# ingonyama-zk/icicle

Measured on NVIDIA H100. Metric: bn254_g1_msm_points_per_s, higher is better.
Workload: dtype u32 limbs (254-bit modular integers, Montgomery arithmetic in IMAD.WIDE chains)

## Files before the change

### icicle_b200/api.py

```python
import copy
import ctypes as C
import enum

import numpy as np

from . import capi
from .capi import IcicleError, MsmConfigC, NttConfigC, VecOpsConfigC, lib, check


class Field(enum.IntEnum):
    BN254_FR = 0
    BN254_FQ = 1
    BLS12_381_FR = 2
    BLS12_381_FQ = 3
    BLS12_377_FR = 4
    BLS12_377_FQ = 5
    BW6_761_FQ = 6
    STARK252 = 7
    BABYBEAR = 8
    KOALABEAR = 9
    M31 = 10
    GOLDILOCKS = 11
    BABYBEAR_EXT4 = 12
    KOALABEAR_EXT4 = 13


FIELD_NAMES = {Field.BN254_FR: "bn254_fr", Field.BN254_FQ: "bn254_fq", Field.BLS12_381_FR: "bls12_381_fr",
               Field.BLS12_381_FQ: "bls12_381_fq", Field.BLS12_377_FR: "bls12_377_fr", Field.BLS12_377_FQ: "bls12_377_fq",
               Field.BW6_761_FQ: "bw6_761_fq", Field.STARK252: "stark252", Field.BABYBEAR: "babybear", Field.KOALABEAR: "koalabear", Field.M31: "m31",
               Field.GOLDILOCKS: "goldilocks"}


class Curve(enum.IntEnum):
    BN254_G1 = 0
    BN254_G2 = 1
    BLS12_381_G1 = 2
    BLS12_381_G2 = 3
    BLS12_377_G1 = 4
    BLS12_377_G2 = 5
    BW6_761_G1 = 6
    BW6_761_G2 = 7
    GRUMPKIN = 8


class NTTDir(enum.IntEnum):
    kForward = 0
    kInverse = 1


class Ordering(enum.IntEnum):
    kNN = 0
    kNR = 1
    kRN = 2
    kRR = 3
    kNM = 4
    kMN = 5


class VecOp(enum.IntEnum):
    ADD = 0
    SUB = 1
    MUL = 2
    ACCUMULATE = 3
    SCALAR_ADD_VEC = 4
    SCALAR_SUB_VEC = 5
    SCALAR_MUL_VEC = 6


def field_limbs(field):
    return lib.b200_field_bytes(int(field)) // 4


def scalar_field(curve):
    return Field(lib.b200_curve_scalar_field(int(curve)))


def affine_limbs(curve):
    return lib.b200_curve_affine_bytes(int(curve)) // 4


def projective_limbs(curve):
    return lib.b200_curve_projective_bytes(int(curve)) // 4


def _is_torch(x):
    return type(x).__module__.startswith("torch")


def is_on_device(x):
    return _is_torch(x) and x.is_cuda


def _ptr(x):
    if _is_torch(x):
        if not x.is_contiguous():
            raise ValueError("device/host tensors must be contiguous")
        return x.data_ptr(), bool(x.is_cuda), x
    a = np.ascontiguousarray(x)
    return a.ctypes.data, False, a


def _out_ptr(x):
    if _is_torch(x):
        return _ptr(x)
    if not isinstance(x, np.ndarray) or not x.flags.c_contiguous or not x.flags.writeable or x.dtype.itemsize != 4:
        raise ValueError("output buffers must be writeable C-contiguous numpy arrays of a 32-bit dtype (uint32 limbs)")
    return x.ctypes.data, False, x


def _stream_handle(stream):
    if stream is None:
        return None
    if hasattr(stream, "cuda_stream"):
        return stream.cuda_stream
    return int(stream)


def device_empty(n_limbs_total, device=None):
    import torch
    return torch.empty(int(n_limbs_total), dtype=torch.int32, device=device or "cuda")


def to_device(host_array, device=None, stream=None):
    import torch
    a = np.ascontiguousarray(host_array, dtype=np.uint32)
    t = torch.empty(a.size, dtype=torch.int32, device=device or "cuda")
    check(lib.b200_copy_to_device(t.data_ptr(), a.ctypes.data, a.nbytes, _stream_handle(stream), 0), "copy_to_device")
    return t.view(*a.shape)


def to_host(dev_tensor, shape=None):
    n = dev_tensor.numel() * dev_tensor.element_size() // 4
    out = np.empty(n, dtype=np.uint32)
    check(lib.b200_copy_to_host(out.ctypes.data, dev_tensor.data_ptr(), out.nbytes, None, 0), "copy_to_host")
    return out.reshape(shape if shape is not None else tuple(dev_tensor.shape))


def set_device(device_id):
    check(lib.b200_set_device(int(device_id)), "set_device")


def get_device_count():
    n = C.c_int(0)
    check(lib.b200_get_device_count(C.byref(n)), "get_device_count")
    return n.value


class MSMConfig:

    def __init__(self, **kw):
        self.stream = None
        self.precompute_factor = 1
        self.c = 0
        self.bitsize = 0
        self.batch_size = 1
        self.are_points_shared_in_batch = True
        self.are_scalars_on_device = False
        self.are_scalars_montgomery_form = False
        self.are_points_on_device = False
        self.are_points_montgomery_form = False
        self.are_results_on_device = False
        self.is_async = False
        self.ext = {}
        for k, v in kw.items():
            if not hasattr(self, k):
                raise TypeError(f"MSMConfig has no field {k}")
            setattr(self, k, v)

    def _c(self):
        c = MsmConfigC()
        lib.b200_msm_default_config(C.byref(c))
        c.stream = _stream_handle(self.stream)
        for k in ("precompute_factor", "c", "bitsize", "batch_size"):
            setattr(c, k, int(getattr(self, k)))
        for k in ("are_points_shared_in_batch", "are_scalars_on_device", "are_scalars_montgomery_form", "are_points_on_device",
                  "are_points_montgomery_form", "are_results_on_device", "is_async"):
            setattr(c, k, 1 if getattr(self, k) else 0)
        c.ext_large_bucket_factor = int(self.ext.get("large_bucket_factor", 0))
        c.ext_nof_chunks = int(self.ext.get("nof_chunks", 0))
        c.ext_is_big_triangle = int(bool(self.ext.get("is_big_triangle", False)))
        return c


def default_msm_config():
    return MSMConfig()


def msm(curve, scalars, bases, msm_size, config=None, results=None):
    cfg = copy.copy(config) if config else MSMConfig()
    sp, s_dev, _ks = _ptr(scalars)
    bp, b_dev, _kb = _ptr(bases)
    cfg.are_scalars_on_device = s_dev
    cfg.are_points_on_device = b_dev
    if results is None:
        if cfg.are_results_on_device:
            results = device_empty(cfg.batch_size * projective_limbs(curve)).view(cfg.batch_size, -1)
        else:
            results = np.zeros((cfg.batch_size, projective_limbs(curve)), dtype=np.uint32)
    rp, r_dev, _kr = _out_ptr(results)
    cfg.are_results_on_device = r_dev
    c = cfg._c()
    check(lib.b200_msm(int(curve), sp, bp, int(msm_size), C.byref(c), rp), "msm")
    return results


def msm_precompute_bases(curve, bases, nof_bases, config, output=None):
    cfg = copy.copy(config)
    bp, b_dev, _kb = _ptr(bases)
    cfg.are_points_on_device = b_dev
    if output is None:
        n = nof_bases * cfg.precompute_factor
        output = (device_empty(n * affine_limbs(curve)).view(n, -1) if cfg.are_results_on_device
                  else np.zeros((n, affine_limbs(curve)), dtype=np.uint32))
    op, o_dev, _ko = _out_ptr(output)
    cfg.are_results_on_device = o_dev
    c = cfg._c()
    check(lib.b200_msm_precompute_bases(int(curve), bp, int(nof_bases), C.byref(c), op), "msm_precompute_bases")
    return output


def ec_sum(curve, points, n, config=None, output=None):
    cfg = config or VecOpsConfig()
    fn, ap, op, c, output = _unary("b200_ec_sum", curve, points, 1, projective_limbs(curve), cfg, output)
    check(fn(int(curve), ap, int(n), C.byref(c), op), "ec_sum")
    return output


def msm_choose_c(curve, msm_size, config=None):
    c = (config or MSMConfig())._c()
    return lib.b200_msm_choose_c(int(curve), int(msm_size), C.byref(c))


def msm_pair_levels(curve, msm_size, c=0, config=None):
    cfg = (config or MSMConfig(c=c))._c()
    return lib.b200_msm_pair_levels(int(curve), int(msm_size), C.byref(cfg))


def shard_range(total, parts, index):
    b, c = C.c_uint64(0), C.c_uint64(0)
    lib.b200_shard_range(int(total), int(parts), int(index), C.byref(b), C.byref(c))
    return b.value, b.value + c.value


def _device_ids(n_devices, device_ids):
    if device_ids is None:
        return int(n_devices), None
    arr = (C.c_int * len(device_ids))(*[int(d) for d in device_ids])
    return len(device_ids), arr


def msm_multi_gpu(curve, scalars, bases, msm_size, config=None, results=None, n_devices=0, device_ids=None):
    cfg = copy.copy(config) if config else MSMConfig()
    sp, s_dev, _ks = _ptr(scalars)
    bp, b_dev, _kb = _ptr(bases)
    if results is None:
        results = np.zeros((cfg.batch_size, projective_limbs(curve)), dtype=np.uint32)
    rp, r_dev, _kr = _out_ptr(results)
    cfg.are_scalars_on_device, cfg.are_points_on_device, cfg.are_results_on_device = s_dev, b_dev, r_dev
    n, ids = _device_ids(n_devices, device_ids)
    c = cfg._c()
    check(lib.b200_msm_multi_gpu(int(curve), sp, bp, int(msm_size), C.byref(c), rp, n, ids), "msm_multi_gpu")
    return results


def ntt_multi_gpu(field, input, size, direction, config=None, output=None, n_devices=0, device_ids=None):
    cfg = copy.copy(config) if config else NTTConfig()
    ip, i_dev, _ki = _ptr(input)
    if output is None:
        output = np.zeros((size * cfg.batch_size, field_limbs(field)), dtype=np.uint32)
    op, o_dev, _ko = _out_ptr(output)
    cfg.are_inputs_on_device, cfg.are_outputs_on_device = i_dev, o_dev
    n, ids = _device_ids(n_devices, device_ids)
    c = cfg._c()
    check(lib.b200_ntt_multi_gpu(int(field), ip, int(size), int(direction), C.byref(c), op, n, ids), "ntt_multi_gpu")
    return output


class NTTConfig:

    def __init__(self, **kw):
        self.stream = None
        self.coset_gen = None
        self.batch_size = 1
        self.columns_batch = False
        self.ordering = Ordering.kNN
        self.are_inputs_on_device = False
        self.are_outputs_on_device = False
        self.is_async = False
        self.ext = {}
        for k, v in kw.items():
            if not hasattr(self, k):
                raise TypeError(f"NTTConfig has no field {k}")
            setattr(self, k, v)

    def _c(self):
        c = NttConfigC()
        lib.b200_ntt_default_config(C.byref(c))
        c.stream = _stream_handle(self.stream)
        self._coset_keep = None
        if self.coset_gen is not None:
            self._coset_keep = np.ascontiguousarray(self.coset_gen, dtype=np.uint32)
            c.coset_gen = self._coset_keep.ctypes.data
        c.batch_size = int(self.batch_size)
        c.columns_batch = 1 if self.columns_batch else 0
        c.are_inputs_on_device = 1 if self.are_inputs_on_device else 0
        c.are_outputs_on_device = 1 if self.are_outputs_on_device else 0
        c.is_async = 1 if self.is_async else 0
        c.ordering = int(self.ordering)
        c.ext_ntt_algorithm = int(self.ext.get("ntt_algorithm", 0))
        c.ext_fast_twiddles = int(bool(self.ext.get("fast_twiddles", False)))
        return c


def default_ntt_config():
    return NTTConfig()


def ntt_init_domain(field, primitive_root, stream=None):
    r = np.ascontiguousarray(primitive_root, dtype=np.uint32)
    check(lib.b200_ntt_init_domain(int(field), r.ctypes.data, _stream_handle(stream)), "ntt_init_domain")


def ntt_release_domain(field):
    check(lib.b200_ntt_release_domain(int(field)), "ntt_release_domain")


def get_root_of_unity_from_domain(field, logn):
    out = np.zeros(field_limbs(field), dtype=np.uint32)
    check(lib.b200_ntt_get_root_of_unity_from_domain(int(field), int(logn), out.ctypes.data), "get_root_of_unity_from_domain")
    return out


def ntt(field, input, size, direction, config=None, output=None):
    cfg = copy.copy(config) if config else NTTConfig()
    ip, i_dev, _ki = _ptr(input)
    cfg.are_inputs_on_device = i_dev
    if output is None:
        n = size * cfg.batch_size * field_limbs(field)
        output = device_empty(n) if cfg.are_outputs_on_device else np.zeros((size * cfg.batch_size, field_limbs(field)), dtype=np.uint32)
    op, o_dev, _ko = _out_ptr(output)
    cfg.are_outputs_on_device = o_dev
    c = cfg._c()
    check(lib.b200_ntt(int(field), ip, int(size), int(direction), C.byref(c), op), "ntt")
    return output


EXTENSION_DEGREE = 4


def ntt_extension(field, input, size, direction, config=None, output=None):
    cfg = copy.copy(config) if config else NTTConfig()
    ip, i_dev, _ki = _ptr(input)
    cfg.are_inputs_on_device = i_dev
    w = field_limbs(field) * EXTENSION_DEGREE
    if output is None:
        n = size * cfg.batch_size * w
        output = device_empty(n) if cfg.are_outputs_on_device else np.zeros((size * cfg.batch_size, w), dtype=np.uint32)
    op, o_dev, _ko = _out_ptr(output)
    cfg.are_outputs_on_device = o_dev
    c = cfg._c()
    check(lib.b200_ntt_extension(int(field), ip, int(size), int(direction), C.byref(c), op), "ntt_extension")
    return output


def ecntt(curve, input, size, direction, config=None, output=None):
    cfg = copy.copy(config) if config else NTTConfig()
    ip, i_dev, _ki = _ptr(input)
    cfg.are_inputs_on_device = i_dev
    w = projective_limbs(curve)
    if output is None:
        n = size * cfg.batch_size * w
        output = device_empty(n) if cfg.are_outputs_on_device else np.zeros((size * cfg.batch_size, w), dtype=np.uint32)
    op, o_dev, _ko = _out_ptr(output)
    cfg.are_outputs_on_device = o_dev
    c = cfg._c()
    check(lib.b200_ecntt(int(curve), ip, int(size), int(direction), C.byref(c), op), "ecntt")
    return output


class VecOpsConfig:

    def __init__(self, **kw):
        self.stream = None
        self.is_a_on_device = False
        self.is_b_on_device = False
        self.is_result_on_device = False
        self.is_async = False
        self.batch_size = 1
        self.columns_batch = False
        for k, v in kw.items():
            if not hasattr(self, k):
                raise TypeError(f"VecOpsConfig has no field {k}")
            setattr(self, k, v)

    def _c(self):
        c = VecOpsConfigC()
        lib.b200_vec_ops_default_config(C.byref(c))
        c.stream = _stream_handle(self.stream)
        c.is_a_on_device = 1 if self.is_a_on_device else 0
        c.is_b_on_device = 1 if self.is_b_on_device else 0
        c.is_result_on_device = 1 if self.is_result_on_device else 0
        c.is_async = 1 if self.is_async else 0
        c.batch_size = int(self.batch_size)
        c.columns_batch = 1 if self.columns_batch else 0
        return c


def _out_like(field, n_elems, on_device):
    if on_device:
        return device_empty(n_elems * field_limbs(field)).view(n_elems, -1)
    return np.zeros((n_elems, field_limbs(field)), dtype=np.uint32)


def _vec2(field, op, a, b, size, config, output):
    cfg = copy.copy(config) if config else VecOpsConfig()
    ap, a_dev, _ka = _ptr(a)
    bp, b_dev, _kb = _ptr(b)
    cfg.is_a_on_device, cfg.is_b_on_device = a_dev, b_dev
    if op == VecOp.ACCUMULATE:
        ap, a_dev, _ka = _out_ptr(a)
        output, op_ptr = a, ap
    else:
        if output is None:
            output = _out_like(field, size * cfg.batch_size, cfg.is_result_on_device)
        op_ptr, o_dev, _ko = _out_ptr(output)
        cfg.is_result_on_device = o_dev
    c = cfg._c()
    check(lib.b200_vec_op(int(field), int(op), ap, bp, int(size), C.byref(c), op_ptr), f"vec_op({VecOp(op).name})")
    return output


def vector_add(field, a, b, size, config=None, output=None):
    return _vec2(field, VecOp.ADD, a, b, size, config, output)


def vector_sub(field, a, b, size, config=None, output=None):
    return _vec2(field, VecOp.SUB, a, b, size, config, output)


def vector_mul(field, a, b, size, config=None, output=None):
    return _vec2(field, VecOp.MUL, a, b, size, config, output)


def vector_accumulate(field, a, b, size, config=None):
    return _vec2(field, VecOp.ACCUMULATE, a, b, size, config, None)


def scalar_add_vec(field, scalar_a, b, size, config=None, output=None):
    return _vec2(field, VecOp.SCALAR_ADD_VEC, scalar_a, b, size, config, output)


def scalar_sub_vec(field, scalar_a, b, size, config=None, output=None):
    return _vec2(field, VecOp.SCALAR_SUB_VEC, scalar_a, b, size, config, output)


def scalar_mul_vec(field, scalar_a, b, size, config=None, output=None):
    return _vec2(field, VecOp.SCALAR_MUL_VEC, scalar_a, b, size, config, output)


def ext_mixed_mul(ext_field, a, b, size, config=None, output=None):
    cfg = copy.copy(config) if config else VecOpsConfig()
    ap, a_dev, _ka = _ptr(a)
    bp, b_dev, _kb = _ptr(b)
    cfg.is_a_on_device, cfg.is_b_on_device = a_dev, b_dev
    if output is None:
        output = _out_like(ext_field, size * cfg.batch_size, cfg.is_result_on_device)
    op, o_dev, _ko = _out_ptr(output)
    cfg.is_result_on_device = o_dev
    c = cfg._c()
    check(lib.b200_ext_mixed_mul(int(ext_field), ap, bp, int(size), C.byref(c), op), "ext_mixed_mul")
    return output


def _unary(fn_name, field_or_curve, a, n_out_elems, limbs, config, output, *extra):
    cfg = copy.copy(config) if config else VecOpsConfig()
    ap, a_dev, _ka = _ptr(a)
    cfg.is_a_on_device = a_dev
    if output is None:
        output = (device_empty(n_out_elems * limbs).view(n_out_elems, -1) if cfg.is_result_on_device
                  else np.zeros((n_out_elems, limbs), dtype=np.uint32))
    op, o_dev, _ko = _out_ptr(output)
    cfg.is_result_on_device = o_dev
    c = cfg._c()
    fn = getattr(lib, fn_name)
    return fn, ap, op, c, output


def vector_inv(field, a, size, config=None, output=None):
    cfg = config or VecOpsConfig()
    fn, ap, op, c, output = _unary("b200_vector_inv", field, a, size * cfg.batch_size, field_limbs(field), cfg, output)
    check(fn(int(field), ap, int(size), C.byref(c), op), "vector_inv")
    return output


def vector_div(field, a, b, size, config=None, output=None):
    cfg = copy.copy(config) if config else VecOpsConfig()
    ap, a_dev, _ka = _ptr(a)
    bp, b_dev, _kb = _ptr(b)
    cfg.is_a_on_device, cfg.is_b_on_device = a_dev, b_dev
    if output is None:
        output = _out_like(field, size * cfg.batch_size, cfg.is_result_on_device)
    op, o_dev, _ko = _out_ptr(output)
    cfg.is_result_on_device = o_dev
    c = cfg._c()
    check(lib.b200_vector_div(int(field), ap, bp, int(size), C.byref(c), op), "vector_div")
    return output


def vector_sum(field, a, size, config=None, output=None):
    cfg = config or VecOpsConfig()
    fn, ap, op, c, output = _unary("b200_vector_sum", field, a, cfg.batch_size, field_limbs(field), cfg, output)
    check(fn(int(field), ap, int(size), C.byref(c), op), "vector_sum")
    return output


def vector_product(field, a, size, config=None, output=None):
    cfg = config or VecOpsConfig()
    fn, ap, op, c, output = _unary("b200_vector_product", field, a, cfg.batch_size, field_limbs(field), cfg, output)
    check(fn(int(field), ap, int(size), C.byref(c), op), "vector_product")
    return output


def highest_non_zero_idx(field, a, size, config=None):
    cfg = copy.copy(config) if config else VecOpsConfig()
    ap, a_dev, _ka = _ptr(a)
    cfg.is_a_on_device = a_dev
    cfg.is_result_on_device = False
    out = np.zeros(cfg.batch_size, dtype=np.int64)
    c = cfg._c()
    check(lib.b200_highest_non_zero_idx(int(field), ap, int(size), C.byref(c), out.ctypes.data), "highest_non_zero_idx")
    return out


def poly_eval(field, coeffs, coeffs_size, domain, domain_size, config=None, output=None):
    cfg = copy.copy(config) if config else VecOpsConfig()
    cp, c_dev, _kc = _ptr(coeffs)
    dp, d_dev, _kd = _ptr(domain)
    cfg.is_a_on_device, cfg.is_b_on_device = c_dev, d_dev
    if output is None:
        output = _out_like(field, domain_size * cfg.batch_size, cfg.is_result_on_device)
    op, o_dev, _ko = _out_ptr(output)
    cfg.is_result_on_device = o_dev
    c = cfg._c()
    check(lib.b200_poly_eval(int(field), cp, int(coeffs_size), dp, int(domain_size), C.byref(c), op), "poly_eval")
    return output


def poly_division(field, numerator, numerator_size, denominator, denominator_size, q_size, r_size, config=None):
    cfg = copy.copy(config) if config else VecOpsConfig()
    n_p, n_dev, _kn = _ptr(numerator)
    d_p, d_dev, _kd = _ptr(denominator)
    cfg.is_a_on_device, cfg.is_b_on_device, cfg.is_result_on_device = n_dev, d_dev, False
    q = np.zeros((q_size * cfg.batch_size, field_limbs(field)), dtype=np.uint32)
    r = np.zeros((r_size * cfg.batch_size, field_limbs(field)), dtype=np.uint32)
    c = cfg._c()
    check(lib.b200_poly_division(int(field), n_p, int(numerator_size), d_p, int(denominator_size), C.byref(c), q.ctypes.data, int(q_size),
                                 r.ctypes.data, int(r_size)), "poly_division")
    return q, r


def convert_montgomery(field, a, size, is_into, config=None, output=None):
    cfg = config or VecOpsConfig()
    fn, ap, op, c, output = _unary("b200_convert_montgomery", field, a, size * cfg.batch_size, field_limbs(field), cfg, output)
    check(fn(int(field), ap, int(size), 1 if is_into else 0, C.byref(c), op), "convert_montgomery")
    return output


def bit_reverse(field, a, size, config=None, output=None):
    cfg = config or VecOpsConfig()
    fn, ap, op, c, output = _unary("b200_bit_reverse", field, a, size * cfg.batch_size, field_limbs(field), cfg, output)
    check(fn(int(field), ap, int(size), C.byref(c), op), "bit_reverse")
    return output


def matrix_transpose(field, a, rows, cols, config=None, output=None):
    cfg = config or VecOpsConfig()
    fn, ap, op, c, output = _unary("b200_matrix_transpose", field, a, rows * cols * cfg.batch_size, field_limbs(field), cfg, output)
    check(fn(int(field), ap, int(rows), int(cols), C.byref(c), op), "matrix_transpose")
    return output


def slice(field, a, offset, stride, size_in, size_out, config=None, output=None):
    cfg = config or VecOpsConfig()
    fn, ap, op, c, output = _unary("b200_slice", field, a, size_out * cfg.batch_size, field_limbs(field), cfg, output)
    check(fn(int(field), ap, int(offset), int(stride), int(size_in), int(size_out), C.byref(c), op), "slice")
    return output


def affine_convert_montgomery(curve, a, n, is_into, config=None, output=None):
    cfg = config or VecOpsConfig()
    fn, ap, op, c, output = _unary("b200_affine_convert_montgomery", curve, a, n, affine_limbs(curve), cfg, output)
    check(fn(int(curve), ap, int(n), 1 if is_into else 0, C.byref(c), op), "affine_convert_montgomery")
    return output


def projective_convert_montgomery(curve, a, n, is_into, config=None, output=None):
    cfg = config or VecOpsConfig()
    fn, ap, op, c, output = _unary("b200_projective_convert_montgomery", curve, a, n, projective_limbs(curve), cfg, output)
    check(fn(int(curve), ap, int(n), 1 if is_into else 0, C.byref(c), op), "projective_convert_montgomery")
    return output


def set_tuning(name, value):
    check(lib.b200_set_tuning(name.encode(), -1 if value is None else int(value)), f"set_tuning({name})")


def get_tuning(name):
    return int(lib.b200_get_tuning(name.encode()))


def trim_scratch(keep_bytes=0):
    check(lib.b200_trim_scratch(int(keep_bytes)), "trim_scratch")


def launch_count():
    return int(lib.b200_get_launch_count())


def set_profiling(on):
    lib.b200_set_profiling(1 if on else 0)


def last_profile():
    names = C.create_string_buffer(2048)
    ms = (C.c_float * 64)()
    k = lib.b200_get_last_profile(names, 2048, ms, 64)
    parts = names.value.decode().split(",")
    return parts[0], [(parts[1 + i], float(ms[i])) for i in range(k)]
```

### icicle_b200/capi.py

```python
import ctypes as C
import os

_HERE = os.path.dirname(os.path.abspath(__file__))
LIB_PATH = os.environ.get("ICICLE_B200_LIB", os.path.join(_HERE, "libicicle_b200.so"))

ERROR_NAMES = {
    0: "SUCCESS", 1: "INVALID_DEVICE", 2: "OUT_OF_MEMORY", 3: "INVALID_POINTER", 4: "ALLOCATION_FAILED",
    5: "DEALLOCATION_FAILED", 6: "COPY_FAILED", 7: "SYNCHRONIZATION_FAILED", 8: "STREAM_CREATION_FAILED",
    9: "STREAM_DESTRUCTION_FAILED", 10: "API_NOT_IMPLEMENTED", 11: "INVALID_ARGUMENT", 12: "BACKEND_LOAD_FAILED",
    13: "LICENSE_CHECK_ERROR", 14: "UNKNOWN_ERROR",
}


class IcicleError(RuntimeError):
    def __init__(self, code, what):
        self.code = code
        super().__init__(f"{what}: eIcicleError::{ERROR_NAMES.get(code, code)}")


class MsmConfigC(C.Structure):
    _fields_ = [
        ("stream", C.c_void_p), ("precompute_factor", C.c_int), ("c", C.c_int), ("bitsize", C.c_int), ("batch_size", C.c_int),
        ("are_points_shared_in_batch", C.c_uint8), ("are_scalars_on_device", C.c_uint8), ("are_scalars_montgomery_form", C.c_uint8),
        ("are_points_on_device", C.c_uint8), ("are_points_montgomery_form", C.c_uint8), ("are_results_on_device", C.c_uint8),
        ("is_async", C.c_uint8), ("reserved", C.c_uint8),
        ("ext_large_bucket_factor", C.c_int), ("ext_nof_chunks", C.c_int), ("ext_is_big_triangle", C.c_int),
    ]


class NttConfigC(C.Structure):
    _fields_ = [
        ("stream", C.c_void_p), ("coset_gen", C.c_void_p), ("batch_size", C.c_int),
        ("columns_batch", C.c_uint8), ("are_inputs_on_device", C.c_uint8), ("are_outputs_on_device", C.c_uint8), ("is_async", C.c_uint8),
        ("ordering", C.c_int), ("ext_ntt_algorithm", C.c_int), ("ext_fast_twiddles", C.c_int),
    ]


class VecOpsConfigC(C.Structure):
    _fields_ = [
        ("stream", C.c_void_p), ("is_a_on_device", C.c_uint8), ("is_b_on_device", C.c_uint8), ("is_result_on_device", C.c_uint8),
        ("is_async", C.c_uint8), ("batch_size", C.c_int), ("columns_batch", C.c_uint8), ("reserved", C.c_uint8 * 3),
    ]


_vp, _i, _u64, _u32, _sz = C.c_void_p, C.c_int, C.c_uint64, C.c_uint32, C.c_size_t
SYMBOLS = {
    "b200_get_device_count": (_i, [C.POINTER(_i)]),
    "b200_set_device": (_i, [_i]),
    "b200_malloc": (_i, [C.POINTER(_vp), _sz]),
    "b200_malloc_async": (_i, [C.POINTER(_vp), _sz, _vp]),
    "b200_free": (_i, [_vp]),
    "b200_free_async": (_i, [_vp, _vp]),
    "b200_get_available_memory": (_i, [C.POINTER(_sz), C.POINTER(_sz)]),
    "b200_memset": (_i, [_vp, _i, _sz]),
    "b200_memset_async": (_i, [_vp, _i, _sz, _vp]),
    "b200_copy_to_device": (_i, [_vp, _vp, _sz, _vp, _i]),
    "b200_copy_to_host": (_i, [_vp, _vp, _sz, _vp, _i]),
    "b200_copy_device_to_device": (_i, [_vp, _vp, _sz, _vp, _i]),
    "b200_synchronize": (_i, [_vp]),
    "b200_create_stream": (_i, [C.POINTER(_vp)]),
    "b200_destroy_stream": (_i, [_vp]),
    "b200_host_alloc_pinned": (_i, [C.POINTER(_vp), _sz]),
    "b200_host_free_pinned": (_i, [_vp]),
    "b200_field_bytes": (_i, [_i]),
    "b200_curve_scalar_field": (_i, [_i]),
    "b200_curve_affine_bytes": (_i, [_i]),
    "b200_curve_projective_bytes": (_i, [_i]),
    "b200_msm_default_config": (None, [C.POINTER(MsmConfigC)]),
    "b200_msm": (_i, [_i, _vp, _vp, _i, C.POINTER(MsmConfigC), _vp]),
    "b200_msm_precompute_bases": (_i, [_i, _vp, _i, C.POINTER(MsmConfigC), _vp]),
    "b200_ec_sum": (_i, [_i, _vp, _i, C.POINTER(VecOpsConfigC), _vp]),
    "b200_msm_choose_c": (_i, [_i, _i, C.POINTER(MsmConfigC)]),
    "b200_msm_pair_levels": (_i, [_i, _i, C.POINTER(MsmConfigC)]),
    "b200_msm_pipeline_schedule": (_i, [_i, C.POINTER(C.c_uint32), _i]),
    "b200_ntt_default_config": (None, [C.POINTER(NttConfigC)]),
    "b200_ntt_init_domain": (_i, [_i, _vp, _vp]),
    "b200_ntt_release_domain": (_i, [_i]),
    "b200_ntt_get_root_of_unity_from_domain": (_i, [_i, _u64, _vp]),
    "b200_ntt": (_i, [_i, _vp, _i, _i, C.POINTER(NttConfigC), _vp]),
    "b200_ntt_extension": (_i, [_i, _vp, _i, _i, C.POINTER(NttConfigC), _vp]),
    "b200_ecntt": (_i, [_i, _vp, _i, _i, C.POINTER(NttConfigC), _vp]),
    "b200_vec_ops_default_config": (None, [C.POINTER(VecOpsConfigC)]),
    "b200_vec_op": (_i, [_i, _i, _vp, _vp, _u64, C.POINTER(VecOpsConfigC), _vp]),
    "b200_ext_mixed_mul": (_i, [_i, _vp, _vp, _u64, C.POINTER(VecOpsConfigC), _vp]),
    "b200_vector_inv": (_i, [_i, _vp, _u64, C.POINTER(VecOpsConfigC), _vp]),
    "b200_vector_div": (_i, [_i, _vp, _vp, _u64, C.POINTER(VecOpsConfigC), _vp]),
    "b200_vector_sum": (_i, [_i, _vp, _u64, C.POINTER(VecOpsConfigC), _vp]),
    "b200_vector_product": (_i, [_i, _vp, _u64, C.POINTER(VecOpsConfigC), _vp]),
    "b200_highest_non_zero_idx": (_i, [_i, _vp, _u64, C.POINTER(VecOpsConfigC), _vp]),
    "b200_poly_eval": (_i, [_i, _vp, _u64, _vp, _u64, C.POINTER(VecOpsConfigC), _vp]),
    "b200_poly_division": (_i, [_i, _vp, _u64, _vp, _u64, C.POINTER(VecOpsConfigC), _vp, _u64, _vp, _u64]),
    "b200_convert_montgomery": (_i, [_i, _vp, _u64, _i, C.POINTER(VecOpsConfigC), _vp]),
    "b200_bit_reverse": (_i, [_i, _vp, _u64, C.POINTER(VecOpsConfigC), _vp]),
    "b200_matrix_transpose": (_i, [_i, _vp, _u32, _u32, C.POINTER(VecOpsConfigC), _vp]),
    "b200_slice": (_i, [_i, _vp, _u64, _u64, _u64, _u64, C.POINTER(VecOpsConfigC), _vp]),
    "b200_affine_convert_montgomery": (_i, [_i, _vp, _u64, _i, C.POINTER(VecOpsConfigC), _vp]),
    "b200_projective_convert_montgomery": (_i, [_i, _vp, _u64, _i, C.POINTER(VecOpsConfigC), _vp]),
    "b200_get_launch_count": (C.c_longlong, []),
    "b200_set_profiling": (None, [_i]),
    "b200_get_last_profile": (_i, [C.c_char_p, _i, C.POINTER(C.c_float), _i]),
    "b200_msm_multi_gpu": (_i, [_i, _vp, _vp, _i, C.POINTER(MsmConfigC), _vp, _i, C.POINTER(_i)]),
    "b200_ntt_multi_gpu": (_i, [_i, _vp, _i, _i, C.POINTER(NttConfigC), _vp, _i, C.POINTER(_i)]),
    "b200_ntt_dist_phase1": (_i, [_i, _vp, _i, _i, _i, _i, _i, _vp]),
    "b200_ntt_dist_phase2": (_i, [_i, _vp, _vp, _i, _i, _i, _i, _i, _vp]),
    "b200_shard_range": (None, [_u64, _i, _i, C.POINTER(_u64), C.POINTER(_u64)]),
    "b200_set_tuning": (_i, [C.c_char_p, _i]),
    "b200_get_tuning": (_i, [C.c_char_p]),
    "b200_trim_scratch": (_i, [_sz]),
    "b200_version": (C.c_char_p, []),
}


def load(path=LIB_PATH):
    if not os.path.exists(path):
        raise ImportError(
            f"icicle_b200: native library not found at {path}. Build it with `python -c 'import __graft_entry__ as g; g.build()'` "
            "or `make -C icicle_b200/csrc`. There is no CPU fallback.")
    lib = C.CDLL(path)
    for name, (res, args) in SYMBOLS.items():
        fn = getattr(lib, name)
        fn.restype = res
        fn.argtypes = args
    return lib


lib = load()


def check(code, what):
    if code != 0:
        raise IcicleError(code, what)
```

### icicle_b200/csrc/common.cuh

```cuda
#pragma once
#include <cuda_runtime.h>
#include <cstdint>
#include <cstdio>
#include <cstdlib>
#include "../../include/icicle_b200.h"
#include "ff.cuh"
#include "ext.cuh"
#include "ext4.cuh"
#include "goldilocks.cuh"
#include "ec.cuh"

namespace b200 {

#define B200_CUDA_TRY(expr, errcode)                                                                                   \
  do {                                                                                                                 \
    cudaError_t _e = (expr);                                                                                           \
    if (_e != cudaSuccess) {                                                                                           \
      fprintf(stderr, "[icicle_b200] %s:%d %s -> %s\n", __FILE__, __LINE__, #expr, cudaGetErrorString(_e));           \
      return (errcode);                                                                                                \
    }                                                                                                                  \
  } while (0)

static inline int map_alloc_error(cudaError_t e) { return e == cudaErrorMemoryAllocation ? B200_OUT_OF_MEMORY : B200_ALLOCATION_FAILED; }

enum Tune : int {
  T_MSM_PAIR_LEVELS = 0, T_MSM_CHUNK_TARGET, T_MSM_NO_WIDE_LOADS, T_MSM_PIPELINE_MIN, T_MSM_PIPELINE_CHUNKS, T_MSM_NO_PIPELINE,
  T_MSM_STAGING_MB, T_MSM_SORT, T_NTT_GEOM, T_NTT31_OFF, T_NTT_COLUMNS_STRIDED, T_NTT_MAXR, T_NTT_TILES, T_NTT_MAXS, T_NTT31_TMA_OFF, T_COPIER_THREADS,
  T_COUNT
};
int tune(Tune k);

cudaMemPool_t scratch_pool();

struct Scratch {
  void* p = nullptr;
  cudaStream_t s = nullptr;
  Scratch() = default;
  Scratch(const Scratch&) = delete;
  Scratch& operator=(const Scratch&) = delete;
  int alloc(size_t bytes, cudaStream_t stream)
  {
    release();
    s = stream;
    if (bytes == 0) bytes = 16;
    cudaMemPool_t pool = scratch_pool();
    cudaError_t e = pool ? cudaMallocFromPoolAsync(&p, bytes, pool, stream) : cudaMallocAsync(&p, bytes, stream);
    if (e != cudaSuccess) {
      p = nullptr;
      fprintf(stderr, "[icicle_b200] scratch allocation of %zu bytes failed: %s\n", bytes, cudaGetErrorString(e));
      (void)cudaGetLastError();
      return map_alloc_error(e);
    }
    return B200_SUCCESS;
  }
  void release()
  {
    if (p) cudaFreeAsync(p, s);
    p = nullptr;
  }
  ~Scratch() { release(); }
  template <class T>
  T* as() const { return reinterpret_cast<T*>(p); }
};

}
#include "hostcopy.cuh"
namespace b200 {

static inline bool ptr_on_device(const void* p, bool flag)
{
  if (flag) return true;
  cudaPointerAttributes a;
  if (cudaPointerGetAttributes(&a, p) != cudaSuccess) {
    (void)cudaGetLastError();
    return false;
  }
  return a.type == cudaMemoryTypeDevice || a.type == cudaMemoryTypeManaged;
}
static inline bool misaligned16(const void* p) { return (((uintptr_t)p) & 15u) != 0; }

static inline int stage_in(const void*& dev_ptr, const void* src, size_t bytes, bool on_device, cudaStream_t s, Scratch& buf)
{
  on_device = ptr_on_device(src, on_device);
  if (on_device && !misaligned16(src)) {
    dev_ptr = src;
    return B200_SUCCESS;
  }
  int err = buf.alloc(bytes, s);
  if (err) return err;
  dev_ptr = buf.p;
  if (!on_device && bytes >= RING_MIN_BYTES && host_kind(src, false) == HK_PAGEABLE) return ring_h2d(buf.p, src, bytes, s);
  B200_CUDA_TRY(cudaMemcpyAsync(buf.p, src, bytes, on_device ? cudaMemcpyDeviceToDevice : cudaMemcpyHostToDevice, s), B200_COPY_FAILED);
  return B200_SUCCESS;
}
static inline int stage_out(void*& dev_ptr, void* dst, size_t bytes, bool on_device, cudaStream_t s, Scratch& buf)
{
  on_device = ptr_on_device(dst, on_device);
  if (on_device && !misaligned16(dst)) {
    dev_ptr = dst;
    return B200_SUCCESS;
  }
  int err = buf.alloc(bytes, s);
  if (err) return err;
  dev_ptr = buf.p;
  return B200_SUCCESS;
}
static inline int finish_out(void* dst, const void* dev_ptr, size_t bytes, bool on_device, bool is_async, cudaStream_t s)
{
  on_device = ptr_on_device(dst, on_device);
  if (dst != dev_ptr && !on_device && bytes >= RING_MIN_BYTES && host_kind(dst, false) == HK_PAGEABLE) return ring_d2h(dst, dev_ptr, bytes, s);
  if (dst != dev_ptr)
    B200_CUDA_TRY(cudaMemcpyAsync(dst, dev_ptr, bytes, on_device ? cudaMemcpyDeviceToDevice : cudaMemcpyDeviceToHost, s), B200_COPY_FAILED);
  if (!on_device || !is_async) B200_CUDA_TRY(cudaStreamSynchronize(s), B200_SYNCHRONIZATION_FAILED);
  return B200_SUCCESS;
}

extern "C" B200_API void b200_count_launch(int n);
#define B200_LAUNCHED(n) b200_count_launch(n)

struct StageTimer {
  static constexpr int MAX_STAGES = 64;
  cudaEvent_t ev[MAX_STAGES + 1];
  const char* names[MAX_STAGES];
  int n = 0;
  bool on = false;
  cudaStream_t s = nullptr;
  void begin(cudaStream_t stream);
  void mark(const char* name);
  void finish(const char* what);
  ~StageTimer();
};

static inline int num_sms()
{
  static thread_local int cached_dev = -1, cached = 132;
  int dev = 0;
  cudaGetDevice(&dev);
  if (dev != cached_dev) {
    cudaDeviceGetAttribute(&cached, cudaDevAttrMultiProcessorCount, dev);
    cached_dev = dev;
  }
  return cached;
}

#define B200_FIELD_CASE(ID, PARAMS, ...)                                                                               \
  case ID: {                                                                                                           \
    using F = ::b200::Fp<::b200::params::PARAMS>;                                                                      \
    __VA_ARGS__;                                                                                                       \
  } break;

#define B200_EXT4_CASE(ID, PARAMS, ...)                                                                                \
  case ID: {                                                                                                           \
    using F = ::b200::Ext4<::b200::params::PARAMS>;                                                                    \
    __VA_ARGS__;                                                                                                       \
  } break;

#define B200_DISPATCH_FIELD(field, ...)                                                                                \
  switch (field) {                                                                                                     \
    B200_FIELD_CASE(B200_FIELD_BN254_FR, bn254_fr, __VA_ARGS__)                                                        \
    B200_FIELD_CASE(B200_FIELD_BN254_FQ, bn254_fq, __VA_ARGS__)                                                        \
    B200_FIELD_CASE(B200_FIELD_BLS12_381_FR, bls12_381_fr, __VA_ARGS__)                                                \
    B200_FIELD_CASE(B200_FIELD_BLS12_381_FQ, bls12_381_fq, __VA_ARGS__)                                                \
    B200_FIELD_CASE(B200_FIELD_BLS12_377_FR, bls12_377_fr, __VA_ARGS__)                                                \
    B200_FIELD_CASE(B200_FIELD_BLS12_377_FQ, bls12_377_fq, __VA_ARGS__)                                                \
    B200_FIELD_CASE(B200_FIELD_BW6_761_FQ, bw6_761_fq, __VA_ARGS__)                                                    \
    B200_FIELD_CASE(B200_FIELD_STARK252, stark252, __VA_ARGS__)                                                        \
    B200_FIELD_CASE(B200_FIELD_BABYBEAR, babybear, __VA_ARGS__)                                                        \
    B200_FIELD_CASE(B200_FIELD_KOALABEAR, koalabear, __VA_ARGS__)                                                      \
    B200_FIELD_CASE(B200_FIELD_M31, m31, __VA_ARGS__)                                                                  \
    B200_FIELD_CASE(B200_FIELD_GOLDILOCKS, goldilocks, __VA_ARGS__)                                                    \
    B200_EXT4_CASE(B200_FIELD_BABYBEAR_EXT4, babybear, __VA_ARGS__)                                                    \
    B200_EXT4_CASE(B200_FIELD_KOALABEAR_EXT4, koalabear, __VA_ARGS__)                                                  \
  default:                                                                                                             \
    return B200_INVALID_ARGUMENT;                                                                                      \
  }

#define B200_DISPATCH_NTT_FIELD(field, ...)                                                                            \
  switch (field) {                                                                                                     \
    B200_FIELD_CASE(B200_FIELD_BN254_FR, bn254_fr, __VA_ARGS__)                                                        \
    B200_FIELD_CASE(B200_FIELD_BLS12_381_FR, bls12_381_fr, __VA_ARGS__)                                                \
    B200_FIELD_CASE(B200_FIELD_BLS12_377_FR, bls12_377_fr, __VA_ARGS__)                                                \
    B200_FIELD_CASE(B200_FIELD_BLS12_377_FQ, bls12_377_fq, __VA_ARGS__)                                                \
    B200_FIELD_CASE(B200_FIELD_STARK252, stark252, __VA_ARGS__)                                                        \
    B200_FIELD_CASE(B200_FIELD_BABYBEAR, babybear, __VA_ARGS__)                                                        \
    B200_FIELD_CASE(B200_FIELD_KOALABEAR, koalabear, __VA_ARGS__)                                                      \
    B200_FIELD_CASE(B200_FIELD_GOLDILOCKS, goldilocks, __VA_ARGS__)                                                    \
  default:                                                                                                             \
    return B200_API_NOT_IMPLEMENTED;                                                                                   \
  }

static inline int field_limbs(int field)
{
  switch (field) {
  case B200_FIELD_BN254_FR: case B200_FIELD_BN254_FQ: case B200_FIELD_BLS12_381_FR: case B200_FIELD_BLS12_377_FR:
  case B200_FIELD_STARK252: return 8;
  case B200_FIELD_BLS12_381_FQ: case B200_FIELD_BLS12_377_FQ: return 12;
  case B200_FIELD_BW6_761_FQ: return 24;
  case B200_FIELD_BABYBEAR: case B200_FIELD_KOALABEAR: case B200_FIELD_M31: return 1;
  case B200_FIELD_GOLDILOCKS: return 2;
  case B200_FIELD_BABYBEAR_EXT4: case B200_FIELD_KOALABEAR_EXT4: return 4;
  default: return 0;
  }
}

template <class FrParams_, class Base_>
struct CurveT {
  typedef FrParams_ FrParams;
  typedef Fp<FrParams_> Scalar;
  typedef Base_ Base;
};

#define B200_CURVE_CASE(ID, FR, BASE, ...)                                                                             \
  case ID: {                                                                                                           \
    using C = ::b200::CurveT<::b200::params::FR, BASE>;                                                                \
    __VA_ARGS__;                                                                                                       \
  } break;

#define B200_DISPATCH_CURVE(curve, ...)                                                                                \
  switch (curve) {                                                                                                     \
    B200_CURVE_CASE(B200_CURVE_BN254_G1, bn254_fr, ::b200::Fp<::b200::params::bn254_fq>, __VA_ARGS__)                  \
    B200_CURVE_CASE(B200_CURVE_BN254_G2, bn254_fr, ::b200::Fp2<::b200::params::bn254_fq>, __VA_ARGS__)                 \
    B200_CURVE_CASE(B200_CURVE_BLS12_381_G1, bls12_381_fr, ::b200::Fp<::b200::params::bls12_381_fq>, __VA_ARGS__)      \
    B200_CURVE_CASE(B200_CURVE_BLS12_381_G2, bls12_381_fr, ::b200::Fp2<::b200::params::bls12_381_fq>, __VA_ARGS__)     \
    B200_CURVE_CASE(B200_CURVE_BLS12_377_G1, bls12_377_fr, ::b200::Fp<::b200::params::bls12_377_fq>, __VA_ARGS__)      \
    B200_CURVE_CASE(B200_CURVE_BLS12_377_G2, bls12_377_fr, ::b200::Fp2<::b200::params::bls12_377_fq>, __VA_ARGS__)     \
    B200_CURVE_CASE(B200_CURVE_BW6_761_G1, bls12_377_fq, ::b200::Fp<::b200::params::bw6_761_fq>, __VA_ARGS__)          \
    B200_CURVE_CASE(B200_CURVE_BW6_761_G2, bls12_377_fq, ::b200::Fp<::b200::params::bw6_761_fq>, __VA_ARGS__)          \
    B200_CURVE_CASE(B200_CURVE_GRUMPKIN, bn254_fq, ::b200::Fp<::b200::params::bn254_fr>, __VA_ARGS__)                  \
  default:                                                                                                             \
    return B200_INVALID_ARGUMENT;                                                                                      \
  }

}
```

### icicle_b200/csrc/msm.cu

```cuda
#include "../../include/icicle_b200.h"
#include <cstring>
#include <cstdint>

#define DECL(ID)                                                                                                       \
  extern "C" int b200_msm_entry_##ID(const void*, const void*, int, const b200_msm_config*, void*) __attribute__((weak)); \
  extern "C" int b200_msm_precompute_entry_##ID(const void*, int, const b200_msm_config*, void*) __attribute__((weak)); \
  extern "C" int b200_msm_plan_c_entry_##ID(int, const b200_msm_config*) __attribute__((weak));                         \
  extern "C" int b200_msm_plan_levels_entry_##ID(int, const b200_msm_config*) __attribute__((weak));                    \
  extern "C" int b200_ec_sum_entry_##ID(const void*, int, const b200_vec_ops_config*, void*) __attribute__((weak));       \
  extern "C" int b200_ecntt_entry_##ID(const void*, int, int, const b200_ntt_config*, void*, const uint32_t*, const uint32_t*, int) __attribute__((weak));
DECL(0) DECL(1) DECL(2) DECL(3) DECL(4) DECL(5) DECL(6) DECL(8)

#define CASE(ID, TU)                                                                                                   \
  case ID:                                                                                                             \
    if (!b200_msm_entry_##TU) return B200_API_NOT_IMPLEMENTED;
#define ALL_CASES(CALL)                                                                                                \
  switch (curve) {                                                                                                     \
    CASE(0, 0) CALL(0);                                                                                                \
    CASE(1, 1) CALL(1);                                                                                                \
    CASE(2, 2) CALL(2);                                                                                                \
    CASE(3, 3) CALL(3);                                                                                                \
    CASE(4, 4) CALL(4);                                                                                                \
    CASE(5, 5) CALL(5);                                                                                                \
    CASE(6, 6) CALL(6);                                                                                                \
    CASE(7, 6) CALL(6);                 \
    CASE(8, 8) CALL(8);                                                                                                \
  default:                                                                                                             \
    return B200_INVALID_ARGUMENT;                                                                                      \
  }

extern "C" {

__attribute__((visibility("default"))) void b200_msm_default_config(b200_msm_config* cfg)
{
  memset(cfg, 0, sizeof(*cfg));
  cfg->precompute_factor = 1;
  cfg->batch_size = 1;
  cfg->are_points_shared_in_batch = 1;
}

__attribute__((visibility("default"))) int
b200_msm(int curve, const void* scalars, const void* bases, int msm_size, const b200_msm_config* cfg, void* results)
{
  if (!cfg || !scalars || !bases || !results) return B200_INVALID_POINTER;
#define CALL(TU) return b200_msm_entry_##TU(scalars, bases, msm_size, cfg, results)
  ALL_CASES(CALL)
#undef CALL
}

__attribute__((visibility("default"))) int
b200_msm_precompute_bases(int curve, const void* input_bases, int nof_bases, const b200_msm_config* cfg, void* output_bases)
{
  if (!cfg || !input_bases || !output_bases) return B200_INVALID_POINTER;
#define CALL(TU) return b200_msm_precompute_entry_##TU(input_bases, nof_bases, cfg, output_bases)
  ALL_CASES(CALL)
#undef CALL
}

__attribute__((visibility("default"))) int
b200_ec_sum(int curve, const void* points, int n, const b200_vec_ops_config* cfg, void* out)
{
  if (!cfg || !points || !out) return B200_INVALID_POINTER;
#define CALL(TU) return b200_ec_sum_entry_##TU(points, n, cfg, out)
  ALL_CASES(CALL)
#undef CALL
}

static int curve_scalar_field(int curve)
{
  switch (curve) {
  case B200_CURVE_BN254_G1: return B200_FIELD_BN254_FR;
  case B200_CURVE_BLS12_381_G1: return B200_FIELD_BLS12_381_FR;
  case B200_CURVE_BLS12_377_G1: return B200_FIELD_BLS12_377_FR;
  case B200_CURVE_BW6_761_G1: return B200_FIELD_BLS12_377_FQ;
  default: return -1;
  }
}
extern "C" int b200_internal_ntt_domain(int field, const uint32_t** tw, const uint32_t** aux, int* max_log);

__attribute__((visibility("default"))) int
b200_ecntt(int curve, const void* input, int size, int dir, const b200_ntt_config* cfg, void* output)
{
  if (!cfg || !input || !output) return B200_INVALID_POINTER;
  const int field = curve_scalar_field(curve);
  if (field < 0) return B200_API_NOT_IMPLEMENTED;
  const uint32_t *tw = nullptr, *aux = nullptr;
  int dom_log = 0;
  int err = b200_internal_ntt_domain(field, &tw, &aux, &dom_log);
  if (err) return err;
#define CALL(TU) return b200_ecntt_entry_##TU(input, size, dir, cfg, output, tw, aux, dom_log)
  ALL_CASES(CALL)
#undef CALL
}

__attribute__((visibility("default"))) int b200_msm_choose_c(int curve, int msm_size, const b200_msm_config* cfg)
{
  if (!cfg) return -1;
#define CALL(TU) return b200_msm_plan_c_entry_##TU(msm_size, cfg)
  ALL_CASES(CALL)
#undef CALL
}

__attribute__((visibility("default"))) int b200_msm_pair_levels(int curve, int msm_size, const b200_msm_config* cfg)
{
  if (!cfg) return -1;
#define CALL(TU) return b200_msm_plan_levels_entry_##TU(msm_size, cfg)
  ALL_CASES(CALL)
#undef CALL
}

}
```

### icicle_b200/csrc/msm_impl.cuh

```cuda
#pragma once
#include "common.cuh"
#include "msm_pairs.cuh"
#include "msm_sort.cuh"
#include <cub/device/device_radix_sort.cuh>
#include <cub/device/device_scan.cuh>
#include <cstdlib>
#include <cstring>
#include <algorithm>
#include <atomic>
#include <memory>
#include <thread>
#include <vector>

namespace b200 { namespace msm {

constexpr int MSM_THREADS = 128;
constexpr uint32_t SIGN_BIT = 0x80000000u;

template <class F>
struct alignas(16) AffineRaw {
  uint32_t w[2 * F::N];
};

template <class F>
B200_D Affine<F> load_affine(const uint32_t* p, bool wide = false)
{
  return {load_el_gather<F>(p, wide), load_el_gather<F>(p + F::N, wide)};
}
template <class F>
B200_D XYZZ<F> load_xyzz(const uint32_t* p)
{
  return {load_el<F>(p), load_el<F>(p + F::N), load_el<F>(p + 2 * F::N), load_el<F>(p + 3 * F::N)};
}
template <class F>
B200_D void store_xyzz(uint32_t* p, const XYZZ<F>& a)
{
  store_el(p, a.x);
  store_el(p + F::N, a.y);
  store_el(p + 2 * F::N, a.zz);
  store_el(p + 3 * F::N, a.zzz);
}

struct MsmPlan {
  int c;
  int bits;
  int nwin;
  int pf;
  int nbm;
  uint32_t bm_buckets;
};

template <class S>
__global__ void __launch_bounds__(256) k_digits(
  const uint32_t* __restrict__ scalars, uint32_t n, uint32_t batch_local, MsmPlan pl, bool scalars_mont, bool shared_points,
  uint32_t* __restrict__ keys, uint32_t* __restrict__ vals, uint32_t sentinel)
{
  uint64_t g = (uint64_t)blockIdx.x * blockDim.x + threadIdx.x;
  if (g >= (uint64_t)n * batch_local) return;
  const uint32_t b = (uint32_t)(g / n), i = (uint32_t)(g % n);
  S s = load_fp<S>(scalars + g * S::N);
  if (scalars_mont) s = s.from_mont();
  const uint32_t c = pl.c, half = 1u << (c - 1), full = 1u << c;
  uint32_t carry = 0;
  const uint64_t ent_base = (uint64_t)b * pl.nwin * n;
  const uint32_t pt_base = shared_points ? 0u : b * n * pl.pf;
  for (int w = 0; w < pl.nwin; w++) {
    const uint32_t lsb = w * c;
    uint32_t raw = 0;
    if (lsb < (uint32_t)pl.bits) {
      const uint32_t limb = lsb >> 5, off = lsb & 31;
      uint64_t two = s.v[limb];
      if (limb + 1 < S::N) two |= (uint64_t)s.v[limb + 1] << 32;
      raw = (uint32_t)(two >> off) & (full - 1);
      const uint32_t avail = pl.bits - lsb;
      if (avail < c) raw &= (1u << avail) - 1;
    }
    raw += carry;
    uint32_t mag, neg;
    if (raw > half) {
      mag = full - raw;
      neg = 1;
      carry = 1;
    } else {
      mag = raw;
      neg = 0;
      carry = 0;
    }
    const uint32_t j = w / pl.nbm, bm = w % pl.nbm;
    uint32_t key = sentinel;
    if (mag) key = (b * pl.nbm + bm) * half + (mag - 1);
    const uint64_t e = ent_base + (uint64_t)w * n + i;
    keys[e] = key;
    vals[e] = (pt_base + i * pl.pf + j) | (neg ? SIGN_BIT : 0u);
  }
}

template <class S>
__global__ void __launch_bounds__(256) k_digits_rank(
  const uint32_t* __restrict__ scalars, uint32_t n, uint32_t batch_local, MsmPlan pl, bool scalars_mont, uint32_t* __restrict__ keys,
  uint32_t* __restrict__ ranks, uint32_t* __restrict__ cnt)
{
  uint64_t g = (uint64_t)blockIdx.x * blockDim.x + threadIdx.x;
  if (g >= (uint64_t)n * batch_local) return;
  const uint32_t b = (uint32_t)(g / n), i = (uint32_t)(g % n);
  S s = load_fp<S>(scalars + g * S::N);
  if (scalars_mont) s = s.from_mont();
  const uint32_t c = pl.c, half = 1u << (c - 1), full = 1u << c;
  uint32_t carry = 0;
  const uint64_t ent_base = (uint64_t)b * pl.nwin * n;
  for (int w = 0; w < pl.nwin; w++) {
    const uint32_t lsb = w * c;
    uint32_t raw = 0;
    if (lsb < (uint32_t)pl.bits) {
      const uint32_t limb = lsb >> 5, off = lsb & 31;
      uint64_t two = s.v[limb];
      if (limb + 1 < S::N) two |= (uint64_t)s.v[limb + 1] << 32;
      raw = (uint32_t)(two >> off) & (full - 1);
      const uint32_t avail = pl.bits - lsb;
      if (avail < c) raw &= (1u << avail) - 1;
    }
    raw += carry;
    uint32_t mag, neg;
    if (raw > half) {
      mag = full - raw;
      neg = SORT_SIGN_BIT;
      carry = 1;
    } else {
      mag = raw;
      neg = 0;
      carry = 0;
    }
    const uint32_t bm = w % pl.nbm;
    uint32_t key = SORT_DROPPED, rk = 0;
    if (mag) {
      key = (b * pl.nbm + bm) * half + (mag - 1);
      rk = atomicAdd(cnt + key, 1u) | neg;
    }
    const uint64_t e = ent_base + (uint64_t)w * n + i;
    keys[e] = key;
    ranks[e] = rk;
  }
}

constexpr uint32_t P_EMPTY = 0xffffffffu;

template <class F, bool DIRECT>
__global__ void __launch_bounds__(MSM_THREADS) k_accumulate(
  const uint32_t* __restrict__ keys, const uint32_t* __restrict__ vals, uint64_t n_entries, const uint32_t* __restrict__ n_dev, uint32_t slice,
  uint32_t sentinel, const uint32_t* __restrict__ points, uint32_t* __restrict__ buckets, uint32_t* __restrict__ pkey,
  uint32_t* __restrict__ pflag, uint32_t* __restrict__ ppt, uint64_t n_slices, bool wide)
{
  constexpr int AW = 2 * F::N, XW = 4 * F::N;
  const uint64_t t = (uint64_t)blockIdx.x * blockDim.x + threadIdx.x;
  if (t >= n_slices) return;
  if (n_dev) n_entries = *n_dev;
  const uint64_t beg = t * slice;
  const uint64_t end = (beg + slice < n_entries) ? beg + slice : n_entries;
  pkey[2 * t] = P_EMPTY;
  pkey[2 * t + 1] = P_EMPTY;
  if (beg >= n_entries) return;

  uint32_t cur = keys[beg];
  if (cur == sentinel) return;
  bool run_starts_here = (beg == 0) || (keys[beg - 1] != cur);
  int slot = 0;
  XYZZ<F> acc = XYZZ<F>::inf();

  uint32_t v = DIRECT ? (uint32_t)beg : vals[beg];
  Affine<F> nxt = load_affine<F>(points + (uint64_t)(v & ~SIGN_BIT) * AW, wide);
  bool nxt_neg = !DIRECT && (v & SIGN_BIT) != 0;

  for (uint64_t e = beg; e < end; e++) {
    Affine<F> p = nxt;
    const bool neg = nxt_neg;
    uint32_t knext = sentinel;
    if (e + 1 < n_entries) knext = keys[e + 1];
    if (e + 1 < end && knext != sentinel) {
      uint32_t v2 = DIRECT ? (uint32_t)(e + 1) : vals[e + 1];
      nxt = load_affine<F>(points + (uint64_t)(v2 & ~SIGN_BIT) * AW, wide);
      nxt_neg = !DIRECT && (v2 & SIGN_BIT) != 0;
    }
    if (neg) p.y = p.y.neg();
    acc.add_affine(p);

    const bool last_in_slice = (e + 1 == end);
    if (knext != cur || last_in_slice) {
      const bool run_ends_here = (knext != cur);
      if (run_starts_here && run_ends_here) {
        store_xyzz<F>(buckets + (uint64_t)cur * XW, acc);
      } else {
        const uint64_t ps = 2 * t + slot;
        pkey[ps] = cur;
        pflag[ps] = (run_starts_here ? 1u : 0u) | (run_ends_here ? 2u : 0u);
        store_xyzz<F>(ppt + ps * XW, acc);
      }
      if (last_in_slice || knext == sentinel) return;
      cur = knext;
      run_starts_here = true;
      slot = 1;
      acc = XYZZ<F>::inf();
    }
  }
}

template <class F>
__global__ void __launch_bounds__(MSM_THREADS) k_reduce_partials(
  const uint32_t* __restrict__ in_key, const uint32_t* __restrict__ in_flag, const uint32_t* __restrict__ in_pt, uint64_t n_in,
  uint32_t seg, uint32_t* __restrict__ out_key, uint32_t* __restrict__ out_flag, uint32_t* __restrict__ out_pt, uint64_t n_threads,
  uint32_t* __restrict__ buckets)
{
  constexpr int XW = 4 * F::N;
  const uint64_t t = (uint64_t)blockIdx.x * blockDim.x + threadIdx.x;
  if (t >= n_threads) return;
  out_key[2 * t] = P_EMPTY;
  out_key[2 * t + 1] = P_EMPTY;
  const uint64_t beg = t * seg;
  const uint64_t end = (beg + seg < n_in) ? beg + seg : n_in;
  bool active = false, started = false;
  uint32_t cur = 0;
  int slot = 0;
  XYZZ<F> acc = XYZZ<F>::inf();
  for (uint64_t j = beg; j < end; j++) {
    const uint32_t key = in_key[j];
    if (key == P_EMPTY) continue;
    const uint32_t fl = in_flag[j];
    XYZZ<F> o = load_xyzz<F>(in_pt + j * XW);
    if (!active) {
      acc = o;
      cur = key;
      started = (fl & 1u) != 0;
      active = true;
    } else {
      acc.add(o);
    }
    if (fl & 2u) {
      if (started) {
        store_xyzz<F>(buckets + (uint64_t)cur * XW, acc);
      } else {
        const uint64_t ps = 2 * t + slot;
        out_key[ps] = cur;
        out_flag[ps] = 2u;
        store_xyzz<F>(out_pt + ps * XW, acc);
      }
      slot = 1;
      active = false;
    }
  }
  if (active) {
    const uint64_t ps = 2 * t + slot;
    out_key[ps] = cur;
    out_flag[ps] = started ? 1u : 0u;
    store_xyzz<F>(out_pt + ps * XW, acc);
  }
}

template <class F>
__global__ void __launch_bounds__(MSM_THREADS) k_resolve(
  const uint32_t* __restrict__ pkey, const uint32_t* __restrict__ pflag, const uint32_t* __restrict__ ppt, uint64_t n_slots,
  uint32_t* __restrict__ buckets)
{
  constexpr int XW = 4 * F::N;
  const uint64_t j = (uint64_t)blockIdx.x * blockDim.x + threadIdx.x;
  if (j >= n_slots) return;
  const uint32_t key = pkey[j];
  if (key == P_EMPTY) return;
  const uint32_t fl = pflag[j];
  if (!(fl & 1u)) return;
  XYZZ<F> acc = load_xyzz<F>(ppt + j * XW);
  if (!(fl & 2u)) {
    for (uint64_t k = j + 1; k < n_slots; k++) {
      if (pkey[k] == P_EMPTY) continue;
      XYZZ<F> o = load_xyzz<F>(ppt + k * XW);
      acc.add(o);
      if (pflag[k] & 2u) break;
    }
  }
  store_xyzz<F>(buckets + (uint64_t)key * XW, acc);
}

template <class F>
__global__ void __launch_bounds__(MSM_THREADS) k_bucket_chunks(
  const uint32_t* __restrict__ buckets, uint32_t n_modules, uint32_t nb_log, uint32_t chunk_log, uint32_t* __restrict__ out)
{
  constexpr int XW = 4 * F::N;
  const uint64_t t = (uint64_t)blockIdx.x * blockDim.x + threadIdx.x;
  const uint32_t chunks_per_module_log = nb_log - chunk_log;
  if (t >= ((uint64_t)n_modules << chunks_per_module_log)) return;
  const uint32_t g = (uint32_t)(t & ((1ull << chunks_per_module_log) - 1));
  const uint64_t first = t << chunk_log;
  const uint32_t L = 1u << chunk_log;
  XYZZ<F> line = XYZZ<F>::inf(), tri = XYZZ<F>::inf();
  for (int k = (int)L - 1; k >= 0; k--) {
    XYZZ<F> b = load_xyzz<F>(buckets + (first + k) * XW);
    line.add(b);
    tri.add(line);
  }
  uint32_t off = g << chunk_log;
  if (off) {
    XYZZ<F> acc = XYZZ<F>::inf();
    for (int bit = 31 - __clz(off); bit >= 0; bit--) {
      acc = acc.dbl();
      if ((off >> bit) & 1) acc.add(line);
    }
    tri.add(acc);
  }
  store_xyzz<F>(out + t * XW, tri);
}

template <class F>
__global__ void __launch_bounds__(MSM_THREADS) k_sum_groups(const uint32_t* __restrict__ in, uint32_t* __restrict__ out, uint64_t n_out, uint32_t k)
{
  constexpr int XW = 4 * F::N;
  const uint64_t i = (uint64_t)blockIdx.x * blockDim.x + threadIdx.x;
  if (i >= n_out) return;
  XYZZ<F> acc = load_xyzz<F>(in + i * k * XW);
  for (uint32_t j = 1; j < k; j++) {
    XYZZ<F> o = load_xyzz<F>(in + (i * k + j) * XW);
    acc.add(o);
  }
  store_xyzz<F>(out + i * XW, acc);
}

template <class F>
__global__ void k_final(const uint32_t* __restrict__ module_sums, uint32_t nbm, uint32_t c, uint32_t batch, uint32_t* __restrict__ results)
{
  constexpr int XW = 4 * F::N;
  const uint32_t b = blockIdx.x * blockDim.x + threadIdx.x;
  if (b >= batch) return;
  XYZZ<F> acc = load_xyzz<F>(module_sums + ((uint64_t)b * nbm + (nbm - 1)) * XW);
  for (int m = (int)nbm - 2; m >= 0; m--) {
    for (uint32_t k = 0; k < c; k++) acc = acc.dbl();
    XYZZ<F> o = load_xyzz<F>(module_sums + ((uint64_t)b * nbm + m) * XW);
    acc.add(o);
  }
  Projective<F> pr = acc.to_projective();
  uint32_t* o = results + (uint64_t)b * 3 * F::N;
  store_el(o, pr.x.from_mont());
  store_el(o + F::N, pr.y.from_mont());
  store_el(o + 2 * F::N, pr.z.from_mont());
}

template <class B>
__global__ void __launch_bounds__(256) k_to_mont(const uint32_t* __restrict__ in, uint32_t* __restrict__ out, uint64_t n)
{
  for (uint64_t i = (uint64_t)blockIdx.x * blockDim.x + threadIdx.x; i < n; i += (uint64_t)gridDim.x * blockDim.x)
    store_fp<B>(out + i * B::N, load_fp<B>(in + i * B::N).to_mont());
}

template <class F>
__global__ void __launch_bounds__(MSM_THREADS) k_precompute(
  const uint32_t* __restrict__ in, uint32_t n, uint32_t pf, uint32_t shift, bool in_mont, bool out_mont, uint32_t* __restrict__ out)
{
  constexpr int AW = 2 * F::N;
  const uint64_t i = (uint64_t)blockIdx.x * blockDim.x + threadIdx.x;
  if (i >= n) return;
  Affine<F> p = load_affine<F>(in + i * AW);
  store_el(out + (i * pf) * AW, p.x);
  store_el(out + (i * pf) * AW + F::N, p.y);
  if (!in_mont) {
    p.x = p.x.to_mont();
    p.y = p.y.to_mont();
  }
  XYZZ<F> q = XYZZ<F>::from_affine(p);
  for (uint32_t j = 1; j < pf; j++) {
    for (uint32_t k = 0; k < shift; k++) q = q.dbl();
    F x = F::zero(), y = F::zero();
    if (!q.is_inf()) {
      F zi = inv_el(q.zzz);
      F zi2 = F::sqr(zi);
      x = q.x * F::sqr(q.zz) * zi2;
      y = q.y * zi;
    }
    if (!out_mont) {
      x = x.from_mont();
      y = y.from_mont();
    }
    store_el(out + (i * pf + j) * AW, x);
    store_el(out + (i * pf + j) * AW + F::N, y);
  }
}

inline int ilog2_ceil(uint64_t x)
{
  int l = 0;
  while ((1ull << l) < x) l++;
  return l;
}

inline int auto_c(int msm_size, int bits, int pf)
{
  double best = 1e300;
  int best_c = 8;
  for (int c = 4; c <= 24; c++) {
    int nwin = (bits + 1 + c - 1) / c;
    int nbm = (nwin + pf - 1) / pf;
    double acc = (double)msm_size * nwin;
    double red = 1.4 * 3.0 * (double)nbm * (double)(1u << (c - 1));
    double cost = acc + red;
    if (cost < best) {
      best = cost;
      best_c = c;
    }
  }
  return best_c;
}

template <class C>
MsmPlan make_plan(int msm_size, const b200_msm_config* cfg)
{
  MsmPlan pl;
  typedef typename C::Scalar S;
  pl.bits = (cfg->bitsize > 0 && cfg->bitsize <= S::P::BITS) ? cfg->bitsize : S::P::BITS;
  pl.pf = cfg->precompute_factor > 0 ? cfg->precompute_factor : 1;
  pl.c = cfg->c > 0 ? cfg->c : auto_c(msm_size, pl.bits, pl.pf);
  if (pl.c < 2) pl.c = 2;
  if (pl.c > 24) pl.c = 24;
  pl.nwin = (pl.bits + 1 + pl.c - 1) / pl.c;
  pl.nbm = (pl.nwin + pl.pf - 1) / pl.pf;
  pl.bm_buckets = 1u << (pl.c - 1);
  return pl;
}

inline int batch_chunk(uint32_t n, const MsmPlan& pl, int batch, bool shared, const b200_msm_config* cfg, size_t coord_bytes = 32)
{
  const uint64_t ent_per_msm = (uint64_t)n * pl.nwin;
  uint64_t max_entries = 1ull << 30;
  if (batch > 1 && ent_per_msm * 2 <= max_entries) {
    size_t free_b = 0, total_b = 0;
    if (cudaMemGetInfo(&free_b, &total_b) == cudaSuccess) {
      const uint64_t per_entry = 16 + (uint64_t)(2.25 * (double)coord_bytes * 2);
      max_entries = std::max<uint64_t>(ent_per_msm, std::min<uint64_t>(max_entries, (uint64_t)(0.45 * (double)free_b) / per_entry));
    } else {
      (void)cudaGetLastError();
    }
  }
  int chunk = (int)std::max<uint64_t>(1, std::min<uint64_t>((uint64_t)batch, max_entries / std::max<uint64_t>(ent_per_msm, 1)));
  if (cfg->ext_nof_chunks > 0) chunk = std::min(chunk, std::max(1, (batch + cfg->ext_nof_chunks - 1) / cfg->ext_nof_chunks));
  if (!shared) {
    while (chunk > 1 && (uint64_t)chunk * n * pl.pf >= (1ull << 31)) chunk--;
  }
  return chunk;
}

inline int choose_pair_levels(uint64_t max_ent, uint64_t max_buckets)
{
  int levels = 0;
  const double avg_run = (double)max_ent / (double)std::max<uint64_t>(max_buckets, 1);
  if (max_ent >= (1ull << 26) && avg_run >= 8.0) {
    while ((8 << levels) <= avg_run && levels < 5) levels++;
  }
  if (tune(T_MSM_PAIR_LEVELS) >= 0) levels = std::min(8, tune(T_MSM_PAIR_LEVELS));
  return levels;
}

enum : int { MSM_ACC = 1, MSM_RED = 2, MSM_ALL = 3 };

template <class C>
int msm_core(const void* d_scal, const uint32_t* pts_m, uint32_t n, const MsmPlan& pl, int batch, bool shared, const b200_msm_config* cfg,
             void* d_res, cudaStream_t s, StageTimer& prof, uint32_t* ext_bkt = nullptr, int phases = MSM_ALL)
{
  typedef typename C::Scalar S;
  typedef typename C::Base F;
  constexpr int AW = 2 * F::N, XW = 4 * F::N, PW = 3 * F::N;
  int err;
  const uint64_t ent_per_msm = (uint64_t)n * pl.nwin;
  int chunk = batch_chunk(n, pl, batch, shared, cfg, (size_t)F::BYTES);
  if ((uint64_t)n * pl.pf >= (1ull << 31) || ent_per_msm >= (1ull << 32)) return B200_INVALID_ARGUMENT;

  const uint64_t max_ent = ent_per_msm * chunk;
  const uint64_t max_modules = (uint64_t)pl.nbm * chunk;
  const uint64_t max_buckets = max_modules << (pl.c - 1);
  if (max_buckets >= 0xfffffff0ull) return B200_INVALID_ARGUMENT;

  const uint64_t target_threads = (uint64_t)num_sms() * 2048;
  uint32_t slice = (uint32_t)std::min<uint64_t>(128, std::max<uint64_t>(8, max_ent / target_threads));
  const uint64_t max_slices = (max_ent + slice - 1) / slice;

  int chunk_target = 16;
  if (tune(T_MSM_CHUNK_TARGET) >= 0) chunk_target = std::max(10, std::min(22, tune(T_MSM_CHUNK_TARGET)));
  int chunk_log = std::max(0, std::min(7, (pl.c - 1 + ilog2_ceil(max_modules)) - chunk_target));
  if (chunk_log > pl.c - 1) chunk_log = pl.c - 1;
  const uint64_t max_chunks = max_buckets >> chunk_log;

  if (ext_bkt && (batch != 1 || chunk != 1)) return B200_INVALID_ARGUMENT;
  const bool do_acc = (phases & MSM_ACC) != 0, do_red = (phases & MSM_RED) != 0;
  Scratch s_k0, s_k1, s_v0, s_v1, s_cub, s_bkt, s_pkey, s_pflag, s_ppt, s_pkey2, s_pflag2, s_ppt2, s_red0, s_red1, s_cnt0, s_off0;
  ScanScratch scan_sc;
  size_t cub_bytes = 0;
  const bool use_cub = tune(T_MSM_SORT) == 1 || (tune(T_MSM_SORT) != 2 && max_ent > (1ull << 25));
  if (do_acc) {
    if ((err = s_k0.alloc(max_ent * 4, s))) return err;
    if ((err = s_k1.alloc(max_ent * 4, s))) return err;
    if ((err = s_v0.alloc(max_ent * 4, s))) return err;
    if ((err = s_v1.alloc(max_ent * 4, s))) return err;
    if (use_cub) {
      cub::DoubleBuffer<uint32_t> dk(s_k0.as<uint32_t>(), s_k1.as<uint32_t>()), dv(s_v0.as<uint32_t>(), s_v1.as<uint32_t>());
      cub::DeviceRadixSort::SortPairs(nullptr, cub_bytes, dk, dv, (int64_t)max_ent, 0, 32, s);
      if ((err = s_cub.alloc(cub_bytes, s))) return err;
    } else {
      if ((err = s_cnt0.alloc((size_t)(max_buckets + 1) * 4, s))) return err;
      if ((err = s_off0.alloc((size_t)(max_buckets + 1) * 4, s))) return err;
    }
    if ((err = scan_sc.prepare(max_buckets + 1, s))) return err;
    if ((err = s_pkey.alloc(max_slices * 2 * 4, s))) return err;
    if ((err = s_pflag.alloc(max_slices * 2 * 4, s))) return err;
    if ((err = s_ppt.alloc(max_slices * 2 * XW * 4, s))) return err;
    const uint64_t max_slots2 = 2 * ((max_slices * 2 + 15) / 16) + 2;
    if ((err = s_pkey2.alloc(max_slots2 * 4, s))) return err;
    if ((err = s_pflag2.alloc(max_slots2 * 4, s))) return err;
    if ((err = s_ppt2.alloc(max_slots2 * XW * 4, s))) return err;
  }
  if (!ext_bkt && (err = s_bkt.alloc(max_buckets * XW * 4, s))) return err;
  uint32_t* const bkt = ext_bkt ? ext_bkt : s_bkt.as<uint32_t>();
  if (do_red) {
    if ((err = s_red0.alloc(std::max<uint64_t>(max_chunks, 1) * XW * 4, s))) return err;
    if ((err = s_red1.alloc(std::max<uint64_t>(max_chunks / 2 + 1, 1) * XW * 4, s))) return err;
  }

  int levels = do_acc ? choose_pair_levels(max_ent, max_buckets) : 0;
  constexpr uint32_t PAIR_J = 32, INV_G = 64;
  const uint32_t nb_max = (uint32_t)max_buckets;
  uint64_t cap[10];
  cap[0] = max_ent;
  for (int l = 0; l < levels; l++) cap[l + 1] = cap[l] / 2 + nb_max + 1;
  Scratch s_off[2], s_cnt, s_lvl[2], s_lkey[2], s_pbuf, s_tree, s_tpre;
  uint64_t tree_m[8];
  int tree_levels = 0;
  uint64_t tree_total = 0;
  if (levels > 0) {
    uint64_t cap_max = cap[0];
    for (int l = 1; l < levels; l++) cap_max = std::max(cap_max, cap[l]);
    uint64_t m = (((cap_max + 1) / 2 + (uint64_t)PAIR_J * PAIR_THREADS - 1) / ((uint64_t)PAIR_J * PAIR_THREADS)) * PAIR_THREADS;
    for (;;) {
      tree_m[tree_levels++] = m;
      tree_total += m;
      if (m <= INV_G) break;
      m = (m + INV_G - 1) / INV_G;
    }
    bool ok = true;
    for (int b = 0; b < 2 && ok; b++) {
      ok = ok && !s_off[b].alloc(((size_t)nb_max + 1) * 4, s);
      if (b < levels) {
        ok = ok && !s_lvl[b].alloc((size_t)cap[b + 1] * AW * 4, s);
        ok = ok && !s_lkey[b].alloc((size_t)cap[b + 1] * 4, s);
      }
    }
    ok = ok && !s_cnt.alloc(((size_t)nb_max + 1) * 4, s) &&
         !s_pbuf.alloc(((size_t)cap[0] / 2 + 1) * F::BYTES, s) && !s_tree.alloc((size_t)tree_total * F::BYTES, s) &&
         !s_tpre.alloc((size_t)tree_total * F::BYTES, s);
    if (!ok) {
      levels = 0;
      for (int b = 0; b < 2; b++) { s_off[b].release(); s_lvl[b].release(); s_lkey[b].release(); }
      s_cnt.release(); s_pbuf.release(); s_tree.release(); s_tpre.release();
    }
  }
  if (levels > 0) {
    uint32_t sl = (uint32_t)std::min<uint64_t>(128, std::max<uint64_t>(8, cap[levels] / target_threads));
    while ((cap[levels] + sl - 1) / sl > max_slices) sl++;
    slice = sl;
  }

  for (int b0 = 0; b0 < batch; b0 += chunk) {
    const int bl = std::min(chunk, batch - b0);
    const uint64_t n_ent = ent_per_msm * bl;
    const uint32_t n_modules = (uint32_t)pl.nbm * bl;
    const uint64_t n_buckets = (uint64_t)n_modules << (pl.c - 1);
    const uint32_t sentinel = (uint32_t)n_buckets;
    const uint32_t* sc = (const uint32_t*)d_scal + (uint64_t)b0 * n * S::N;
    const uint32_t* pts = pts_m + (shared ? 0 : (uint64_t)b0 * n * pl.pf * AW);
    const bool pts_wide = (((uintptr_t)pts) & 31u) == 0 && (F::BYTES % 32 == 0) && tune(T_MSM_NO_WIDE_LOADS) <= 0;

    if (do_acc) {
    const uint32_t nb = (uint32_t)n_buckets;
    const uint32_t* sorted_k;
    const uint32_t* sorted_v;
    const uint32_t* n_live = nullptr;
    uint32_t* off_first = (levels > 0) ? s_off[0].as<uint32_t>() : s_off0.as<uint32_t>();
    uint32_t acc_sentinel = sentinel;
    if (use_cub) {
      uint64_t th = (uint64_t)n * bl;
      k_digits<S><<<(unsigned)((th + 255) / 256), 256, 0, s>>>(
        sc, n, (uint32_t)bl, pl, cfg->are_scalars_montgomery_form, shared, s_k0.as<uint32_t>(), s_v0.as<uint32_t>(), sentinel); B200_LAUNCHED(1);
      B200_CUDA_TRY(cudaGetLastError(), B200_UNKNOWN_ERROR);
      prof.mark("digits");
      cub::DoubleBuffer<uint32_t> dk(s_k0.as<uint32_t>(), s_k1.as<uint32_t>()), dv(s_v0.as<uint32_t>(), s_v1.as<uint32_t>());
      const int key_bits = std::max(1, ilog2_ceil((uint64_t)sentinel + 1));
      B200_CUDA_TRY(cub::DeviceRadixSort::SortPairs(s_cub.p, cub_bytes, dk, dv, (int64_t)n_ent, 0, key_bits, s), B200_UNKNOWN_ERROR);
      sorted_k = dk.Current();
      sorted_v = dv.Current();
      if (levels > 0) {
        k_bounds<<<(nb + 1 + 255) / 256, 256, 0, s>>>(sorted_k, (uint32_t)n_ent, nb, off_first); B200_LAUNCHED(1);
      }
      prof.mark("sort");
    } else {
      B200_CUDA_TRY(cudaMemsetAsync(s_cnt0.p, 0, ((size_t)nb + 1) * 4, s), B200_UNKNOWN_ERROR);
      uint64_t th = (uint64_t)n * bl;
      k_digits_rank<S><<<(unsigned)((th + 255) / 256), 256, 0, s>>>(
        sc, n, (uint32_t)bl, pl, cfg->are_scalars_montgomery_form, s_k0.as<uint32_t>(), s_v0.as<uint32_t>(), s_cnt0.as<uint32_t>()); B200_LAUNCHED(1);
      B200_CUDA_TRY(cudaGetLastError(), B200_UNKNOWN_ERROR);
      prof.mark("digits");
      if ((err = exclusive_scan_u32(s_cnt0.as<uint32_t>(), off_first, (uint64_t)nb + 1, scan_sc, s))) return err;
      k_scatter<<<(unsigned)((n_ent + 255) / 256), 256, 0, s>>>(s_k0.as<uint32_t>(), s_v0.as<uint32_t>(), n_ent, n, (uint32_t)pl.nwin, (uint32_t)pl.nbm,
                                                               (uint32_t)pl.pf, shared, off_first, s_k1.as<uint32_t>(), s_v1.as<uint32_t>()); B200_LAUNCHED(1);
      B200_CUDA_TRY(cudaGetLastError(), B200_UNKNOWN_ERROR);
      sorted_k = s_k1.as<uint32_t>();
      sorted_v = s_v1.as<uint32_t>();
      n_live = off_first + nb;
      acc_sentinel = 0xffffffffu;
      prof.mark("sort");
    }
    B200_CUDA_TRY(cudaMemsetAsync(bkt, 0, n_buckets * XW * 4, s), B200_UNKNOWN_ERROR);
    uint64_t n_slices;
    if (levels == 0) {
      n_slices = (n_ent + slice - 1) / slice;
      k_accumulate<F, false><<<(unsigned)((n_slices + MSM_THREADS - 1) / MSM_THREADS), MSM_THREADS, 0, s>>>(
        sorted_k, sorted_v, n_ent, n_live, slice, acc_sentinel, pts, bkt, s_pkey.as<uint32_t>(),
        s_pflag.as<uint32_t>(), s_ppt.as<uint32_t>(), n_slices, pts_wide); B200_LAUNCHED(1);
      B200_CUDA_TRY(cudaGetLastError(), B200_UNKNOWN_ERROR);
    } else {
      const unsigned gb = (nb + 1 + 255) / 256;
      uint64_t capl = n_ent;
      const uint32_t *lk = sorted_k, *lp = pts;
      uint64_t lcap = 0;
      uint4* pbuf = s_pbuf.as<uint4>();
      const uint64_t pcap = cap[0] / 2 + 1;
      for (int l = 0; l < levels; l++) {
        uint32_t* off_c = s_off[l & 1].as<uint32_t>();
        uint32_t* off_n = s_off[(l + 1) & 1].as<uint32_t>();
        k_pair_counts<<<gb, 256, 0, s>>>(off_c, nb, s_cnt.as<uint32_t>()); B200_LAUNCHED(1);
        if ((err = exclusive_scan_u32(s_cnt.as<uint32_t>(), off_n, (uint64_t)nb + 1, scan_sc, s))) return err;
        const uint64_t nq = (capl + 1) / 2;
        const unsigned gp = (unsigned)((nq + (uint64_t)PAIR_J * PAIR_THREADS - 1) / ((uint64_t)PAIR_J * PAIR_THREADS));
        const uint32_t nthr = gp * PAIR_THREADS;
        uint32_t* tree = s_tree.as<uint32_t>();
        uint32_t* tpre = s_tpre.as<uint32_t>();
        uint32_t* out_p = s_lvl[l & 1].as<uint32_t>();
        uint32_t* out_k = s_lkey[l & 1].as<uint32_t>();
        const uint64_t ocap = cap[(l & 1) + 1];
        const bool last = (l + 1 == levels);
        if (l == 0) {
          PairSrc<F, true> src = {lk, sorted_v, lp, 0, pts_wide};
          k_pair_prefix<F, true><<<gp, PAIR_THREADS, 0, s>>>(src, off_c, nb, PAIR_J, pbuf, pcap, tree);
        } else {
          PairSrc<F, false> src = {lk, nullptr, lp, lcap, false};
          k_pair_prefix<F, false><<<gp, PAIR_THREADS, 0, s>>>(src, off_c, nb, PAIR_J, pbuf, pcap, tree);
        }
        B200_LAUNCHED(1);
        {
          uint64_t m[8], o[8];
          int R = 0;
          uint64_t mm = nthr, oo = 0;
          for (;;) {
            m[R] = mm; o[R] = oo; R++;
            if (mm <= INV_G) break;
            oo += mm;
            mm = (mm + INV_G - 1) / INV_G;
          }
          for (int r = 0; r + 1 < R; r++) {
            k_inv_up<F><<<(unsigned)((m[r + 1] + 127) / 128), 128, 0, s>>>(
              tree + o[r] * F::N, (uint32_t)m[r], INV_G, tpre + o[r] * F::N, tree + o[r + 1] * F::N, (uint32_t)m[r + 1]); B200_LAUNCHED(1);
          }
          k_inv_top<F><<<1, 32, 0, s>>>(tree + o[R - 1] * F::N, (uint32_t)m[R - 1], tpre + o[R - 1] * F::N); B200_LAUNCHED(1);
          for (int r = R - 2; r >= 0; r--) {
            k_inv_down<F><<<(unsigned)((m[r + 1] + 127) / 128), 128, 0, s>>>(
              tree + o[r] * F::N, (uint32_t)m[r], INV_G, tpre + o[r] * F::N, tree + o[r + 1] * F::N, (uint32_t)m[r + 1]); B200_LAUNCHED(1);
          }
        }
        if (l == 0) {
          PairSrc<F, true> src = {lk, sorted_v, lp, 0, pts_wide};
          if (last) k_pair_apply<F, true, false><<<gp, PAIR_THREADS, 0, s>>>(src, off_c, off_n, nb, PAIR_J, pbuf, pcap, tree, out_p, ocap, out_k);
          else k_pair_apply<F, true, true><<<gp, PAIR_THREADS, 0, s>>>(src, off_c, off_n, nb, PAIR_J, pbuf, pcap, tree, out_p, ocap, out_k);
        } else {
          PairSrc<F, false> src = {lk, nullptr, lp, lcap, false};
          if (last) k_pair_apply<F, false, false><<<gp, PAIR_THREADS, 0, s>>>(src, off_c, off_n, nb, PAIR_J, pbuf, pcap, tree, out_p, ocap, out_k);
          else k_pair_apply<F, false, true><<<gp, PAIR_THREADS, 0, s>>>(src, off_c, off_n, nb, PAIR_J, pbuf, pcap, tree, out_p, ocap, out_k);
        }
        B200_LAUNCHED(1);
        B200_CUDA_TRY(cudaGetLastError(), B200_UNKNOWN_ERROR);
        lk = out_k; lp = out_p; lcap = ocap;
        capl = capl / 2 + nb + 1;
      }
      prof.mark("pair_levels");
      n_slices = (capl + slice - 1) / slice;
      k_accumulate<F, true><<<(unsigned)((n_slices + MSM_THREADS - 1) / MSM_THREADS), MSM_THREADS, 0, s>>>(
        lk, nullptr, 0, s_off[levels & 1].as<uint32_t>() + nb, slice, 0xffffffffu, lp, bkt, s_pkey.as<uint32_t>(),
        s_pflag.as<uint32_t>(), s_ppt.as<uint32_t>(), n_slices, true); B200_LAUNCHED(1);
      B200_CUDA_TRY(cudaGetLastError(), B200_UNKNOWN_ERROR);
    }
    prof.mark("accumulate");
    {
      uint32_t *ik = s_pkey.as<uint32_t>(), *ifl = s_pflag.as<uint32_t>(), *ipt = s_ppt.as<uint32_t>();
      uint32_t *ok = s_pkey2.as<uint32_t>(), *ofl = s_pflag2.as<uint32_t>(), *opt = s_ppt2.as<uint32_t>();
      uint64_t n_slots = 2 * n_slices;
      const uint32_t seg = 16;
      while (n_slots > 512) {
        const uint64_t nt = (n_slots + seg - 1) / seg;
        k_reduce_partials<F><<<(unsigned)((nt + MSM_THREADS - 1) / MSM_THREADS), MSM_THREADS, 0, s>>>(
          ik, ifl, ipt, n_slots, seg, ok, ofl, opt, nt, bkt); B200_LAUNCHED(1);
        B200_CUDA_TRY(cudaGetLastError(), B200_UNKNOWN_ERROR);
        std::swap(ik, ok);
        std::swap(ifl, ofl);
        std::swap(ipt, opt);
        n_slots = 2 * nt;
      }
      k_resolve<F><<<(unsigned)((n_slots + MSM_THREADS - 1) / MSM_THREADS), MSM_THREADS, 0, s>>>(ik, ifl, ipt, n_slots, bkt); B200_LAUNCHED(1);
      B200_CUDA_TRY(cudaGetLastError(), B200_UNKNOWN_ERROR);
    }
    prof.mark("resolve");
    }
    if (!do_red) continue;
    const uint64_t n_chunks = n_buckets >> chunk_log;
    k_bucket_chunks<F><<<(unsigned)((n_chunks + MSM_THREADS - 1) / MSM_THREADS), MSM_THREADS, 0, s>>>(
      bkt, n_modules, (uint32_t)(pl.c - 1), (uint32_t)chunk_log, s_red0.as<uint32_t>()); B200_LAUNCHED(1);
    B200_CUDA_TRY(cudaGetLastError(), B200_UNKNOWN_ERROR);
    uint32_t* cur = s_red0.as<uint32_t>();
    uint32_t* other = s_red1.as<uint32_t>();
    uint64_t per_module = 1ull << (pl.c - 1 - chunk_log);
    while (per_module > 1) {
      const uint32_t k = (uint32_t)std::min<uint64_t>(per_module, 8);
      const uint64_t n_out = (uint64_t)n_modules * (per_module / k);
      k_sum_groups<F><<<(unsigned)((n_out + MSM_THREADS - 1) / MSM_THREADS), MSM_THREADS, 0, s>>>(cur, other, n_out, k); B200_LAUNCHED(1);
      B200_CUDA_TRY(cudaGetLastError(), B200_UNKNOWN_ERROR);
      std::swap(cur, other);
      per_module /= k;
    }
    prof.mark("bucket_reduce");
    k_final<F><<<(bl + 31) / 32, 32, 0, s>>>(cur, (uint32_t)pl.nbm, (uint32_t)pl.c, (uint32_t)bl, (uint32_t*)d_res + (uint64_t)b0 * PW); B200_LAUNCHED(1);
    B200_CUDA_TRY(cudaGetLastError(), B200_UNKNOWN_ERROR);
  }
  return B200_SUCCESS;
}

template <class F>
__global__ void __launch_bounds__(MSM_THREADS) k_bucket_merge(uint32_t* __restrict__ dst, const uint32_t* __restrict__ src, uint64_t n)
{
  constexpr int XW = 4 * F::N;
  const uint64_t i = (uint64_t)blockIdx.x * blockDim.x + threadIdx.x;
  if (i >= n) return;
  XYZZ<F> b = load_xyzz<F>(src + i * XW);
  if (b.is_inf()) return;
  XYZZ<F> a = load_xyzz<F>(dst + i * XW);
  a.add(b);
  store_xyzz<F>(dst + i * XW, a);
}

inline uint32_t pipeline_min_points()
{
  if (tune(T_MSM_PIPELINE_MIN) >= 0) return (uint32_t)std::max(2, tune(T_MSM_PIPELINE_MIN));
  return 1u << 23;
}

inline uint32_t pipeline_schedule(uint32_t n, uint32_t* sizes, uint32_t max_chunks)
{
  const bool tiny_ok = tune(T_MSM_PIPELINE_MIN) >= 0;
  const uint32_t min_chunk = tiny_ok ? 1u : (1u << 20);
  uint32_t k = 0, left = n;
  if (tune(T_MSM_PIPELINE_CHUNKS) > 0) {
    const uint32_t want = (uint32_t)std::max(1, std::min((int)max_chunks, tune(T_MSM_PIPELINE_CHUNKS)));
    const uint32_t each = std::max<uint32_t>((n + want - 1) / want, min_chunk);
    while (left > 0 && k < max_chunks) {
      sizes[k] = (k + 1 == max_chunks) ? left : std::min(each, left);
      left -= sizes[k++];
    }
    return k;
  }
  static const uint32_t shift[6] = {4, 4, 3, 2, 2, 2};
  for (int i = 0; i < 6 && left > 0; i++) {
    uint32_t want = std::max<uint32_t>(n >> shift[i], min_chunk);
    if (i == 5 || left < want + min_chunk) want = left;
    sizes[k] = std::min(want, left);
    left -= sizes[k++];
  }
  return k;
}

inline uint32_t device_chunk_points(const MsmPlan& pl) { return (uint32_t)std::max<uint64_t>(1, (1ull << 30) / (uint64_t)pl.nwin); }

template <class C>
int msm_chunked(const void* scalars, const void* bases, uint32_t n, const b200_msm_config* cfg, void* results, HostKind ks, HostKind kp)
{
  typedef typename C::Scalar S;
  typedef typename C::Base F;
  typedef typename base_fp<F>::type B;
  constexpr int AW = 2 * F::N, XW = 4 * F::N, PW = 3 * F::N;
  constexpr uint32_t MAX_CHUNKS = 32;
  cudaStream_t s = (cudaStream_t)cfg->stream;
  DeviceRes* res = device_res();
  if (!res) return B200_UNKNOWN_ERROR;
  cudaStream_t cs = res->copy_stream;
  b200_msm_config sub = *cfg;
  sub.batch_size = 1;
  const MsmPlan pl = make_plan<C>((int)n, &sub);
  const uint32_t pf = (uint32_t)pl.pf;
  const bool any_host = (ks != HK_DEVICE) || (kp != HK_DEVICE);
  uint32_t csize[MAX_CHUNKS], coff[MAX_CHUNKS];
  uint32_t nchunks;
  if (any_host) {
    nchunks = pipeline_schedule(n, csize, MAX_CHUNKS);
  } else {
    const uint32_t cap = device_chunk_points(pl);
    nchunks = std::min<uint32_t>(MAX_CHUNKS, (n + cap - 1) / cap);
    const uint32_t each = (n + nchunks - 1) / nchunks;
    uint32_t left = n;
    for (uint32_t i = 0; i < nchunks; i++) {
      csize[i] = std::min(each, left);
      left -= csize[i];
    }
    if (left) return B200_INVALID_ARGUMENT;
  }
  uint32_t max_chunk = 0;
  for (uint32_t i = 0, o = 0; i < nchunks; o += csize[i], i++) {
    coff[i] = o;
    max_chunk = std::max(max_chunk, csize[i]);
  }
  const uint64_t n_buckets = (uint64_t)pl.nbm << (pl.c - 1);
  int err;
  Scratch d_s, d_p, d_pm, d_bkt, d_tmp, s_res;
  ChunkArray as, ap;
  as.kind = ks; as.elem_bytes = S::BYTES; as.host = (const uint8_t*)scalars; as.dev = (uint8_t*)const_cast<void*>(scalars);
  ap.kind = kp; ap.elem_bytes = (size_t)pf * AW * 4; ap.host = (const uint8_t*)bases; ap.dev = (uint8_t*)const_cast<void*>(bases);
  if (ks != HK_DEVICE) {
    if ((err = d_s.alloc((size_t)n * S::BYTES, s))) return err;
    as.dev = d_s.as<uint8_t>();
  } else if (misaligned16(scalars)) {
    return B200_INVALID_POINTER;
  }
  if (kp != HK_DEVICE) {
    if ((err = d_p.alloc((size_t)n * ap.elem_bytes, s))) return err;
    ap.dev = d_p.as<uint8_t>();
  } else {
    if (misaligned16(bases)) return B200_INVALID_POINTER;
    if (!cfg->are_points_montgomery_form && (err = d_pm.alloc((size_t)max_chunk * ap.elem_bytes, s))) return err;
  }
  if ((err = d_bkt.alloc((size_t)n_buckets * XW * 4, s))) return err;
  if (nchunks > 1 && (err = d_tmp.alloc((size_t)n_buckets * XW * 4, s))) return err;
  void* d_res;
  if ((err = stage_out(d_res, results, (size_t)PW * 4, cfg->are_results_on_device, s, s_res))) return err;

  PageableCopy pageable;
  cudaEvent_t ready = res->event(0);
  const bool direct_copies = (ks == HK_PINNED) || (kp == HK_PINNED);
  const bool ring_copies = (ks == HK_PAGEABLE) || (kp == HK_PAGEABLE);
  if (any_host) {
    cudaEventRecord(ready, s);
    if (direct_copies) {
      cudaStreamWaitEvent(cs, ready, 0);
      for (uint32_t i = 0; i < nchunks; i++) {
        const size_t off = coff[i], cn = csize[i];
        if (ks == HK_PINNED) cudaMemcpyAsync(as.dev + off * as.elem_bytes, as.host + off * as.elem_bytes, cn * as.elem_bytes, cudaMemcpyHostToDevice, cs);
        if (kp == HK_PINNED) cudaMemcpyAsync(ap.dev + off * ap.elem_bytes, ap.host + off * ap.elem_bytes, cn * ap.elem_bytes, cudaMemcpyHostToDevice, cs);
        cudaEventRecord(res->event(1 + i), cs);
      }
    }
    if (ring_copies) {
      if (ks == HK_PAGEABLE) pageable.add(as, coff, csize, nchunks);
      if (kp == HK_PAGEABLE) pageable.add(ap, coff, csize, nchunks);
      if ((err = pageable.start(res, nchunks, ready))) return err;
    }
  }

  StageTimer prof;
  prof.begin(s);
  int rc = B200_SUCCESS;
  for (uint32_t i = 0; i < nchunks && rc == B200_SUCCESS; i++) {
    const uint32_t off = coff[i], cn = csize[i];
    if (direct_copies) cudaStreamWaitEvent(s, res->event(1 + i), 0);
    if (ring_copies) pageable.wait_chunk(i, s);
    const uint32_t* cp = (const uint32_t*)(ap.dev + (size_t)off * ap.elem_bytes);
    if (!cfg->are_points_montgomery_form) {
      uint32_t* dst = (kp != HK_DEVICE) ? const_cast<uint32_t*>(cp) : d_pm.as<uint32_t>();
      const uint64_t ncoord = (uint64_t)cn * pf * 2 * (F::N / B::N);
      unsigned g = (unsigned)std::min<uint64_t>((ncoord + 255) / 256, (uint64_t)num_sms() * 16);
      k_to_mont<B><<<g, 256, 0, s>>>(cp, dst, ncoord); B200_LAUNCHED(1);
      cp = dst;
    }
    uint32_t* target = (i == 0) ? d_bkt.as<uint32_t>() : d_tmp.as<uint32_t>();
    rc = msm_core<C>(as.dev + (size_t)off * S::BYTES, cp, cn, pl, 1, true, &sub, nullptr, s, prof, target, MSM_ACC);
    if (rc == B200_SUCCESS && i > 0) {
      k_bucket_merge<F><<<(unsigned)((n_buckets + MSM_THREADS - 1) / MSM_THREADS), MSM_THREADS, 0, s>>>(d_bkt.as<uint32_t>(), d_tmp.as<uint32_t>(), n_buckets);
      B200_LAUNCHED(1);
      if (cudaGetLastError() != cudaSuccess) rc = B200_UNKNOWN_ERROR;
      prof.mark("merge");
    }
  }
  if (rc == B200_SUCCESS) rc = msm_core<C>(nullptr, nullptr, max_chunk, pl, 1, true, &sub, d_res, s, prof, d_bkt.as<uint32_t>(), MSM_RED);
  prof.mark("final");
  prof.finish(any_host ? "msm_pipelined" : "msm_chunked");
  pageable.join();
  if (pageable.failed.load()) rc = B200_COPY_FAILED;
  if (rc == B200_SUCCESS && any_host && !(cfg->are_results_on_device && cfg->is_async) && stream_sync_blocking(s) != cudaSuccess) rc = B200_SYNCHRONIZATION_FAILED;
  if (rc == B200_SUCCESS) rc = finish_out(results, d_res, (size_t)PW * 4, cfg->are_results_on_device, cfg->is_async, s);
  if (rc != B200_SUCCESS || any_host) {
    if (direct_copies) cudaStreamSynchronize(cs);
    for (CopierCtx* c : pageable.ctx) cudaStreamSynchronize(c->st);
    if (rc != B200_SUCCESS) cudaStreamSynchronize(s);
  }
  return rc;
}

template <class C>
int msm_impl(const void* scalars, const void* bases, int msm_size, const b200_msm_config* cfg, void* results)
{
  typedef typename C::Scalar S;
  typedef typename C::Base F;
  typedef typename base_fp<F>::type B;
  constexpr int AW = 2 * F::N, XW = 4 * F::N, PW = 3 * F::N;
  cudaStream_t s = (cudaStream_t)cfg->stream;
  const int batch = cfg->batch_size > 0 ? cfg->batch_size : 1;
  if (msm_size <= 0) return B200_INVALID_ARGUMENT;
  const MsmPlan pl = make_plan<C>(msm_size, cfg);
  const uint32_t n = (uint32_t)msm_size;
  if ((uint64_t)n * pl.pf >= (1ull << 31)) return B200_INVALID_ARGUMENT;
  const HostKind ks = host_kind(scalars, cfg->are_scalars_on_device), kp = host_kind(bases, cfg->are_points_on_device);
  if (batch == 1) {
    const bool any_host = (ks != HK_DEVICE) || (kp != HK_DEVICE);
    const bool pipeline = any_host && n >= pipeline_min_points() && tune(T_MSM_NO_PIPELINE) <= 0;
    const bool too_big = !any_host && n > device_chunk_points(pl);
    if (pipeline || too_big || (any_host && n > device_chunk_points(pl))) return msm_chunked<C>(scalars, bases, n, cfg, results, ks, kp);
  }
  const bool shared = cfg->are_points_shared_in_batch || batch == 1;
  const uint64_t n_points = (uint64_t)n * pl.pf * (shared ? 1 : batch);
  int err;

  Scratch s_scal, s_pts, s_pts_m, s_res;
  const void *d_scal, *d_pts;
  void* d_res;
  if ((err = stage_in(d_scal, scalars, (size_t)n * batch * S::BYTES, ks == HK_DEVICE, s, s_scal))) return err;
  if ((err = stage_in(d_pts, bases, (size_t)n_points * AW * 4, kp == HK_DEVICE, s, s_pts))) return err;
  if ((err = stage_out(d_res, results, (size_t)batch * PW * 4, cfg->are_results_on_device, s, s_res))) return err;
  const uint32_t* pts_m = (const uint32_t*)d_pts;
  if (!cfg->are_points_montgomery_form) {
    uint32_t* dst;
    if (d_pts != bases) {
      dst = s_pts.as<uint32_t>();
    } else {
      if ((err = s_pts_m.alloc((size_t)n_points * AW * 4, s))) return err;
      dst = s_pts_m.as<uint32_t>();
    }
    const uint64_t ncoord = n_points * 2 * (F::N / B::N);
    unsigned g = (unsigned)std::min<uint64_t>((ncoord + 255) / 256, (uint64_t)num_sms() * 16);
    k_to_mont<B><<<g, 256, 0, s>>>((const uint32_t*)d_pts, dst, ncoord); B200_LAUNCHED(1);
    B200_CUDA_TRY(cudaGetLastError(), B200_UNKNOWN_ERROR);
    pts_m = dst;
  }

  StageTimer prof;
  prof.begin(s);
  if ((err = msm_core<C>(d_scal, pts_m, n, pl, batch, shared, cfg, d_res, s, prof))) return err;
  prof.mark("final");
  prof.finish("msm");
  return finish_out(results, d_res, (size_t)batch * PW * 4, cfg->are_results_on_device, cfg->is_async, s);
}

template <class C>
int precompute_impl(const void* in, int n, const b200_msm_config* cfg, void* out)
{
  typedef typename C::Base F;
  constexpr int AW = 2 * F::N;
  cudaStream_t s = (cudaStream_t)cfg->stream;
  if (n <= 0) return B200_INVALID_ARGUMENT;
  const MsmPlan pl = make_plan<C>(n, cfg);
  const uint32_t shift = (uint32_t)pl.c * pl.nbm;
  Scratch s_in, s_out;
  const void* d_in;
  void* d_out;
  int err;
  const size_t bytes_in = (size_t)n * AW * 4, bytes_out = bytes_in * pl.pf;
  if ((err = stage_in(d_in, in, bytes_in, cfg->are_points_on_device, s, s_in))) return err;
  if ((err = stage_out(d_out, out, bytes_out, cfg->are_results_on_device, s, s_out))) return err;
  k_precompute<F><<<(n + MSM_THREADS - 1) / MSM_THREADS, MSM_THREADS, 0, s>>>(
    (const uint32_t*)d_in, (uint32_t)n, (uint32_t)pl.pf, shift, cfg->are_points_montgomery_form, cfg->are_points_montgomery_form, (uint32_t*)d_out); B200_LAUNCHED(1);
  B200_CUDA_TRY(cudaGetLastError(), B200_UNKNOWN_ERROR);
  return finish_out(out, d_out, bytes_out, cfg->are_results_on_device, cfg->is_async, s);
}


template <class F>
__global__ void k_proj_sum(const uint32_t* __restrict__ in, uint32_t n, uint32_t* __restrict__ out)
{
  constexpr int PW = 3 * F::N;
  if (blockIdx.x != 0 || threadIdx.x != 0) return;
  XYZZ<F> acc = XYZZ<F>::inf();
  for (uint32_t i = 0; i < n; i++) {
    Projective<F> p = {load_el<F>(in + (uint64_t)i * PW).to_mont(), load_el<F>(in + (uint64_t)i * PW + F::N).to_mont(),
                       load_el<F>(in + (uint64_t)i * PW + 2 * F::N).to_mont()};
    XYZZ<F> q = XYZZ<F>::from_projective(p);
    acc.add(q);
  }
  Projective<F> r = acc.to_projective();
  store_el(out, r.x.from_mont());
  store_el(out + F::N, r.y.from_mont());
  store_el(out + 2 * F::N, r.z.from_mont());
}

template <class C>
int ec_sum_impl(const void* points, int n, const b200_vec_ops_config* cfg, void* out)
{
  typedef typename C::Base F;
  constexpr int PW = 3 * F::N;
  cudaStream_t s = (cudaStream_t)cfg->stream;
  if (n <= 0) return B200_INVALID_ARGUMENT;
  Scratch s_in, s_out;
  const void* d_in;
  void* d_out;
  int err;
  if ((err = stage_in(d_in, points, (size_t)n * PW * 4, cfg->is_a_on_device, s, s_in))) return err;
  if ((err = stage_out(d_out, out, (size_t)PW * 4, cfg->is_result_on_device, s, s_out))) return err;
  k_proj_sum<F><<<1, 32, 0, s>>>((const uint32_t*)d_in, (uint32_t)n, (uint32_t*)d_out); B200_LAUNCHED(1);
  B200_CUDA_TRY(cudaGetLastError(), B200_UNKNOWN_ERROR);
  return finish_out(out, d_out, (size_t)PW * 4, cfg->is_result_on_device, cfg->is_async, s);
}

}}
```

### icicle_b200/csrc/msm_inst.cu

```cuda
#include "msm_impl.cuh"
#include <type_traits>
#include "ecntt.cuh"

#define B200_CAT2(a, b) a##b
#define B200_CAT(a, b) B200_CAT2(a, b)

namespace b200 { namespace msm {
template <int ID> struct CurveOf;
template <> struct CurveOf<B200_CURVE_BN254_G1> { typedef CurveT<params::bn254_fr, Fp<params::bn254_fq>> type; };
template <> struct CurveOf<B200_CURVE_BN254_G2> { typedef CurveT<params::bn254_fr, Fp2<params::bn254_fq>> type; };
template <> struct CurveOf<B200_CURVE_BLS12_381_G1> { typedef CurveT<params::bls12_381_fr, Fp<params::bls12_381_fq>> type; };
template <> struct CurveOf<B200_CURVE_BLS12_381_G2> { typedef CurveT<params::bls12_381_fr, Fp2<params::bls12_381_fq>> type; };
template <> struct CurveOf<B200_CURVE_BLS12_377_G1> { typedef CurveT<params::bls12_377_fr, Fp<params::bls12_377_fq>> type; };
template <> struct CurveOf<B200_CURVE_BLS12_377_G2> { typedef CurveT<params::bls12_377_fr, Fp2<params::bls12_377_fq>> type; };
template <> struct CurveOf<B200_CURVE_BW6_761_G1> { typedef CurveT<params::bls12_377_fq, Fp<params::bw6_761_fq>> type; };
template <> struct CurveOf<B200_CURVE_GRUMPKIN> { typedef CurveT<params::bn254_fq, Fp<params::bn254_fr>> type; };
}}

using namespace b200;
using namespace b200::msm;
typedef CurveOf<B200_MSM_CURVE>::type ThisCurve;

template <class C, bool G1 = std::is_same<typename C::Base, typename base_fp<typename C::Base>::type>::value>
struct EcnttEntry {
  static int run(const void* in, int size, int dir, const b200_ntt_config* cfg, void* out, const uint32_t* tw, const uint32_t* aux, int dom_log)
  {
    return ecntt::ecntt_impl<C>(in, size, dir, cfg, out, tw, aux, dom_log);
  }
};
template <class C>
struct EcnttEntry<C, false> {
  static int run(const void*, int, int, const b200_ntt_config*, void*, const uint32_t*, const uint32_t*, int) { return B200_API_NOT_IMPLEMENTED; }
};

extern "C" {
__attribute__((visibility("hidden"))) int B200_CAT(b200_msm_entry_, B200_MSM_CURVE)(
  const void* scalars, const void* bases, int msm_size, const b200_msm_config* cfg, void* results)
{
  return msm_impl<ThisCurve>(scalars, bases, msm_size, cfg, results);
}
__attribute__((visibility("hidden"))) int B200_CAT(b200_msm_precompute_entry_, B200_MSM_CURVE)(
  const void* in, int n, const b200_msm_config* cfg, void* out)
{
  return precompute_impl<ThisCurve>(in, n, cfg, out);
}
__attribute__((visibility("hidden"))) int B200_CAT(b200_ec_sum_entry_, B200_MSM_CURVE)(
  const void* points, int n, const b200_vec_ops_config* cfg, void* out)
{
  return ec_sum_impl<ThisCurve>(points, n, cfg, out);
}
__attribute__((visibility("hidden"))) int B200_CAT(b200_ecntt_entry_, B200_MSM_CURVE)(
  const void* input, int size, int dir, const b200_ntt_config* cfg, void* output, const uint32_t* tw, const uint32_t* aux, int dom_log)
{
  return EcnttEntry<ThisCurve>::run(input, size, dir, cfg, output, tw, aux, dom_log);
}
#if B200_MSM_CURVE == 0
__attribute__((visibility("default"))) int b200_msm_pipeline_schedule(int msm_size, uint32_t* sizes, int max_chunks)
{
  if (msm_size <= 0 || !sizes || max_chunks <= 0) return -1;
  return (int)pipeline_schedule((uint32_t)msm_size, sizes, (uint32_t)std::min(max_chunks, 32));
}
#endif
__attribute__((visibility("hidden"))) int B200_CAT(b200_msm_plan_c_entry_, B200_MSM_CURVE)(int msm_size, const b200_msm_config* cfg)
{
  return make_plan<ThisCurve>(msm_size, cfg).c;
}
__attribute__((visibility("hidden"))) int B200_CAT(b200_msm_plan_levels_entry_, B200_MSM_CURVE)(int msm_size, const b200_msm_config* cfg)
{
  const MsmPlan pl = make_plan<ThisCurve>(msm_size, cfg);
  const int batch = cfg->batch_size > 0 ? cfg->batch_size : 1;
  const bool shared = cfg->are_points_shared_in_batch || batch == 1;
  const int chunk = batch_chunk((uint32_t)msm_size, pl, batch, shared, cfg, (size_t)ThisCurve::Base::BYTES);
  const uint64_t max_ent = (uint64_t)msm_size * pl.nwin * chunk;
  const uint64_t max_buckets = ((uint64_t)pl.nbm * chunk) << (pl.c - 1);
  return choose_pair_levels(max_ent, max_buckets);
}
}
```

### icicle_b200/csrc/msm_sort.cuh

```cuda
#pragma once
#include "common.cuh"

namespace b200 { namespace msm {

constexpr uint32_t SORT_SIGN_BIT = 0x80000000u;
constexpr uint32_t SORT_DROPPED = 0xffffffffu;

struct MsmPlan;

constexpr int SCAN_BLOCK = 1024;
static __global__ void __launch_bounds__(256) k_scan_block_sums(const uint32_t* __restrict__ in, uint64_t n, uint32_t* __restrict__ block_sums)
{
  __shared__ uint32_t red[8];
  const uint64_t base = (uint64_t)blockIdx.x * SCAN_BLOCK + threadIdx.x * 4;
  uint32_t s = 0;
#pragma unroll
  for (int j = 0; j < 4; j++)
    if (base + j < n) s += in[base + j];
  for (int o = 16; o > 0; o >>= 1) s += __shfl_down_sync(0xffffffffu, s, o);
  if ((threadIdx.x & 31) == 0) red[threadIdx.x >> 5] = s;
  __syncthreads();
  if (threadIdx.x == 0) {
    uint32_t t = 0;
    for (int w = 0; w < 8; w++) t += red[w];
    block_sums[blockIdx.x] = t;
  }
}
static __global__ void __launch_bounds__(1024) k_scan_top(uint32_t* __restrict__ sums, uint32_t m)
{
  __shared__ uint32_t wsum[32];
  __shared__ uint32_t carry;
  if (threadIdx.x == 0) carry = 0;
  __syncthreads();
  for (uint32_t base = 0; base < m; base += 1024) {
    const uint32_t i = base + threadIdx.x;
    const uint32_t v = (i < m) ? sums[i] : 0u;
    uint32_t x = v;
    for (int o = 1; o < 32; o <<= 1) {
      const uint32_t y = __shfl_up_sync(0xffffffffu, x, o);
      if ((int)(threadIdx.x & 31) >= o) x += y;
    }
    if ((threadIdx.x & 31) == 31) wsum[threadIdx.x >> 5] = x;
    __syncthreads();
    if (threadIdx.x < 32) {
      uint32_t w = wsum[threadIdx.x];
      for (int o = 1; o < 32; o <<= 1) {
        const uint32_t y = __shfl_up_sync(0xffffffffu, w, o);
        if ((int)threadIdx.x >= o) w += y;
      }
      wsum[threadIdx.x] = w;
    }
    __syncthreads();
    const uint32_t warp_excl = (threadIdx.x >> 5) ? wsum[(threadIdx.x >> 5) - 1] : 0u;
    const uint32_t incl = x + warp_excl;
    if (i < m) sums[i] = carry + incl - v;
    __syncthreads();
    if (threadIdx.x == 1023) carry += incl;
    __syncthreads();
  }
}
static __global__ void __launch_bounds__(256) k_scan_apply(const uint32_t* __restrict__ in, uint64_t n, const uint32_t* __restrict__ block_excl,
                                                           uint32_t* __restrict__ out)
{
  __shared__ uint32_t wsum[8];
  const uint64_t base = (uint64_t)blockIdx.x * SCAN_BLOCK + threadIdx.x * 4;
  uint32_t v[4];
  uint32_t s = 0;
#pragma unroll
  for (int j = 0; j < 4; j++) {
    v[j] = (base + j < n) ? in[base + j] : 0u;
    s += v[j];
  }
  uint32_t x = s;
  for (int o = 1; o < 32; o <<= 1) {
    const uint32_t y = __shfl_up_sync(0xffffffffu, x, o);
    if ((int)(threadIdx.x & 31) >= o) x += y;
  }
  if ((threadIdx.x & 31) == 31) wsum[threadIdx.x >> 5] = x;
  __syncthreads();
  uint32_t woff = 0;
  for (int w = 0; w < (int)(threadIdx.x >> 5); w++) woff += wsum[w];
  uint32_t run = block_excl[blockIdx.x] + woff + x - s;
#pragma unroll
  for (int j = 0; j < 4; j++) {
    if (base + j < n) out[base + j] = run;
    run += v[j];
  }
}

struct ScanScratch {
  Scratch sums;
  uint32_t blocks = 0;
  int prepare(uint64_t n_max, cudaStream_t s)
  {
    blocks = (uint32_t)((n_max + SCAN_BLOCK - 1) / SCAN_BLOCK);
    return sums.alloc((size_t)std::max<uint32_t>(blocks, 1) * 4, s);
  }
};
static inline int exclusive_scan_u32(const uint32_t* in, uint32_t* out, uint64_t n, ScanScratch& sc, cudaStream_t s)
{
  const uint32_t blocks = (uint32_t)((n + SCAN_BLOCK - 1) / SCAN_BLOCK);
  if (blocks == 0) return B200_SUCCESS;
  k_scan_block_sums<<<blocks, 256, 0, s>>>(in, n, sc.sums.as<uint32_t>()); B200_LAUNCHED(1);
  k_scan_top<<<1, 1024, 0, s>>>(sc.sums.as<uint32_t>(), blocks); B200_LAUNCHED(1);
  k_scan_apply<<<blocks, 256, 0, s>>>(in, n, sc.sums.as<uint32_t>(), out); B200_LAUNCHED(1);
  B200_CUDA_TRY(cudaGetLastError(), B200_UNKNOWN_ERROR);
  return B200_SUCCESS;
}

static __global__ void __launch_bounds__(256) k_scatter(const uint32_t* __restrict__ keys0, const uint32_t* __restrict__ rank0, uint64_t n_ent,
                                                        uint32_t n, uint32_t nwin, uint32_t nbm, uint32_t pf, bool shared_points,
                                                        const uint32_t* __restrict__ off, uint32_t* __restrict__ keys1, uint32_t* __restrict__ vals1)
{
  const uint64_t e = (uint64_t)blockIdx.x * blockDim.x + threadIdx.x;
  if (e >= n_ent) return;
  const uint32_t key = keys0[e];
  if (key == SORT_DROPPED) return;
  const uint32_t r = rank0[e];
  const uint32_t i = (uint32_t)(e % n);
  const uint32_t bw = (uint32_t)(e / n);
  const uint32_t b = bw / nwin, w = bw % nwin;
  const uint32_t val = ((shared_points ? 0u : b * n * pf) + i * pf + w / nbm) | (r & SORT_SIGN_BIT);
  const uint32_t pos = off[key] + (r & ~SORT_SIGN_BIT);
  keys1[pos] = key;
  vals1[pos] = val;
}

}}
```

### icicle_b200/csrc/runtime.cu

```cuda
#include "common.cuh"
#include <cstring>

using namespace b200;

#include <atomic>
#include <mutex>
#include <string>
#include <cctype>
#include <cstdlib>
namespace {
  std::atomic<long long> g_launches{0};
  std::atomic<int> g_profiling{0};
  std::mutex g_prof_mu;
  std::string g_prof_what;
  int g_prof_n = 0;
  char g_prof_names[StageTimer::MAX_STAGES][32];
  float g_prof_ms[StageTimer::MAX_STAGES];
}

namespace {
  const char* const kTuneNames[b200::T_COUNT] = {
    "msm_pair_levels", "msm_chunk_target", "msm_no_wide_loads", "msm_pipeline_min", "msm_pipeline_chunks", "msm_no_pipeline",
    "msm_staging_mb", "msm_sort", "ntt_geom", "ntt31_off", "ntt_columns_strided", "ntt_maxr", "ntt_tiles", "ntt_maxs", "ntt31_tma_off", "copier_threads"};
  std::atomic<int> g_tune[b200::T_COUNT];
  struct TuneInit {
    TuneInit()
    {
      for (int i = 0; i < b200::T_COUNT; i++) {
        std::string env = "B200_";
        for (const char* c = kTuneNames[i]; *c; c++) env += (char)toupper((unsigned char)*c);
        const char* v = getenv(env.c_str());
        g_tune[i].store(v ? atoi(v) : -1);
      }
    }
  } g_tune_init;

  std::mutex g_pool_mu;
  cudaMemPool_t g_pools[64] = {};
  bool g_pool_tried[64] = {};
}

namespace b200 {
  int tune_copier_threads() { return g_tune[T_COPIER_THREADS].load(std::memory_order_relaxed); }
  int tune(Tune k) { return (k >= 0 && k < T_COUNT) ? g_tune[k].load(std::memory_order_relaxed) : -1; }

  cudaMemPool_t scratch_pool()
  {
    int dev = 0;
    if (cudaGetDevice(&dev) != cudaSuccess || dev < 0 || dev >= 64) return nullptr;
    if (g_pool_tried[dev]) return g_pools[dev];
    std::lock_guard<std::mutex> lk(g_pool_mu);
    if (g_pool_tried[dev]) return g_pools[dev];
    cudaMemPoolProps props;
    memset(&props, 0, sizeof(props));
    props.allocType = cudaMemAllocationTypePinned;
    props.handleTypes = cudaMemHandleTypeNone;
    props.location.type = cudaMemLocationTypeDevice;
    props.location.id = dev;
    cudaMemPool_t pool = nullptr;
    if (cudaMemPoolCreate(&pool, &props) == cudaSuccess) {
      uint64_t thresh = UINT64_MAX;
      if (const char* ev = getenv("B200_SCRATCH_RETAIN_MB")) thresh = (uint64_t)atoll(ev) << 20;
      cudaMemPoolSetAttribute(pool, cudaMemPoolAttrReleaseThreshold, &thresh);
      g_pools[dev] = pool;
    } else {
      (void)cudaGetLastError();
      g_pools[dev] = nullptr;
    }
    g_pool_tried[dev] = true;
    return g_pools[dev];
  }

  StageTimer::~StageTimer()
  {
    if (!on) return;
    for (int i = 0; i <= n; i++) cudaEventDestroy(ev[i]);
  }
  void StageTimer::begin(cudaStream_t stream)
  {
    on = g_profiling.load() != 0;
    s = stream;
    n = 0;
    if (!on) return;
    cudaEventCreate(&ev[0]);
    cudaEventRecord(ev[0], s);
  }
  void StageTimer::mark(const char* name)
  {
    if (!on || n >= MAX_STAGES) return;
    names[n] = name;
    cudaEventCreate(&ev[n + 1]);
    cudaEventRecord(ev[n + 1], s);
    n++;
  }
  void StageTimer::finish(const char* what)
  {
    if (!on) return;
    cudaEventSynchronize(ev[n]);
    std::lock_guard<std::mutex> lk(g_prof_mu);
    g_prof_what = what;
    g_prof_n = n;
    for (int i = 0; i < n; i++) {
      cudaEventElapsedTime(&g_prof_ms[i], ev[i], ev[i + 1]);
      strncpy(g_prof_names[i], names[i], 31);
      g_prof_names[i][31] = 0;
    }
    for (int i = 0; i <= n; i++) cudaEventDestroy(ev[i]);
    on = false;
  }
}

extern "C" {

void b200_count_launch(int n) { g_launches.fetch_add(n, std::memory_order_relaxed); }
long long b200_get_launch_count(void) { return g_launches.load(); }
void b200_set_profiling(int on) { g_profiling.store(on); }
int b200_get_last_profile(char* names_out, int names_cap, float* ms_out, int max_stages)
{
  std::lock_guard<std::mutex> lk(g_prof_mu);
  std::string joined = g_prof_what;
  int k = g_prof_n < max_stages ? g_prof_n : max_stages;
  for (int i = 0; i < k; i++) {
    joined += std::string(",") + g_prof_names[i];
    ms_out[i] = g_prof_ms[i];
  }
  if (names_out && names_cap > 0) {
    strncpy(names_out, joined.c_str(), names_cap - 1);
    names_out[names_cap - 1] = 0;
  }
  return k;
}

int b200_set_tuning(const char* name, int value)
{
  if (!name) return B200_INVALID_POINTER;
  if (!strcmp(name, "l2_fetch_granularity")) {
    if (value != 32 && value != 64 && value != 128) return B200_INVALID_ARGUMENT;
    B200_CUDA_TRY(cudaDeviceSetLimit(cudaLimitMaxL2FetchGranularity, (size_t)value), B200_UNKNOWN_ERROR);
    return B200_SUCCESS;
  }
  for (int i = 0; i < b200::T_COUNT; i++) {
    if (!strcmp(name, kTuneNames[i])) {
      g_tune[i].store(value < 0 ? -1 : value);
      return B200_SUCCESS;
    }
  }
  return B200_INVALID_ARGUMENT;
}
int b200_get_tuning(const char* name)
{
  if (!name) return -1;
  for (int i = 0; i < b200::T_COUNT; i++)
    if (!strcmp(name, kTuneNames[i])) return g_tune[i].load();
  return -1;
}

int b200_trim_scratch(size_t keep_bytes)
{
  cudaMemPool_t pool = b200::scratch_pool();
  if (!pool) return B200_SUCCESS;
  B200_CUDA_TRY(cudaDeviceSynchronize(), B200_SYNCHRONIZATION_FAILED);
  B200_CUDA_TRY(cudaMemPoolTrimTo(pool, keep_bytes), B200_DEALLOCATION_FAILED);
  return B200_SUCCESS;
}

const char* b200_version(void) { return "icicle_b200 0.2 (sm_90a; MSM+NTT+vec-ops; C ABI v2)"; }

int b200_get_device_count(int* count)
{
  int n = 0;
  cudaError_t e = cudaGetDeviceCount(&n);
  if (e != cudaSuccess) {
    (void)cudaGetLastError();
    *count = 0;
    return B200_INVALID_DEVICE;
  }
  *count = n;
  return B200_SUCCESS;
}

int b200_set_device(int device_id)
{
  int n = 0;
  if (cudaGetDeviceCount(&n) != cudaSuccess || device_id < 0 || device_id >= n) {
    (void)cudaGetLastError();
    return B200_INVALID_DEVICE;
  }
  B200_CUDA_TRY(cudaSetDevice(device_id), B200_INVALID_DEVICE);
  return B200_SUCCESS;
}

int b200_malloc(void** ptr, size_t bytes)
{
  cudaError_t e = cudaMalloc(ptr, bytes);
  if (e != cudaSuccess) {
    (void)cudaGetLastError();
    *ptr = nullptr;
    return map_alloc_error(e);
  }
  return B200_SUCCESS;
}
int b200_malloc_async(void** ptr, size_t bytes, void* stream)
{
  cudaError_t e = cudaMallocAsync(ptr, bytes, (cudaStream_t)stream);
  if (e != cudaSuccess) {
    (void)cudaGetLastError();
    *ptr = nullptr;
    return map_alloc_error(e);
  }
  return B200_SUCCESS;
}
int b200_free(void* ptr)
{
  B200_CUDA_TRY(cudaFree(ptr), B200_DEALLOCATION_FAILED);
  return B200_SUCCESS;
}
int b200_free_async(void* ptr, void* stream)
{
  B200_CUDA_TRY(cudaFreeAsync(ptr, (cudaStream_t)stream), B200_DEALLOCATION_FAILED);
  return B200_SUCCESS;
}
int b200_get_available_memory(size_t* total, size_t* free_bytes)
{
  B200_CUDA_TRY(cudaMemGetInfo(free_bytes, total), B200_UNKNOWN_ERROR);
  return B200_SUCCESS;
}
int b200_memset(void* ptr, int value, size_t bytes)
{
  B200_CUDA_TRY(cudaMemset(ptr, value, bytes), B200_UNKNOWN_ERROR);
  return B200_SUCCESS;
}
int b200_memset_async(void* ptr, int value, size_t bytes, void* stream)
{
  B200_CUDA_TRY(cudaMemsetAsync(ptr, value, bytes, (cudaStream_t)stream), B200_UNKNOWN_ERROR);
  return B200_SUCCESS;
}
static int copy_impl(void* dst, const void* src, size_t bytes, cudaMemcpyKind kind, void* stream, int is_async)
{
  if (is_async) {
    B200_CUDA_TRY(cudaMemcpyAsync(dst, src, bytes, kind, (cudaStream_t)stream), B200_COPY_FAILED);
  } else {
    B200_CUDA_TRY(cudaMemcpy(dst, src, bytes, kind), B200_COPY_FAILED);
  }
  return B200_SUCCESS;
}
int b200_copy_to_device(void* dst, const void* src, size_t bytes, void* stream, int is_async)
{
  return copy_impl(dst, src, bytes, cudaMemcpyHostToDevice, stream, is_async);
}
int b200_copy_to_host(void* dst, const void* src, size_t bytes, void* stream, int is_async)
{
  return copy_impl(dst, src, bytes, cudaMemcpyDeviceToHost, stream, is_async);
}
int b200_copy_device_to_device(void* dst, const void* src, size_t bytes, void* stream, int is_async)
{
  return copy_impl(dst, src, bytes, cudaMemcpyDeviceToDevice, stream, is_async);
}
int b200_synchronize(void* stream)
{
  if (stream) {
    B200_CUDA_TRY(cudaStreamSynchronize((cudaStream_t)stream), B200_SYNCHRONIZATION_FAILED);
  } else {
    B200_CUDA_TRY(cudaDeviceSynchronize(), B200_SYNCHRONIZATION_FAILED);
  }
  return B200_SUCCESS;
}
int b200_create_stream(void** stream)
{
  cudaStream_t s;
  B200_CUDA_TRY(cudaStreamCreateWithFlags(&s, cudaStreamNonBlocking), B200_STREAM_CREATION_FAILED);
  *stream = (void*)s;
  return B200_SUCCESS;
}
int b200_destroy_stream(void* stream)
{
  B200_CUDA_TRY(cudaStreamDestroy((cudaStream_t)stream), B200_STREAM_DESTRUCTION_FAILED);
  return B200_SUCCESS;
}
int b200_host_alloc_pinned(void** ptr, size_t bytes)
{
  cudaError_t e = cudaHostAlloc(ptr, bytes, cudaHostAllocDefault);
  if (e != cudaSuccess) {
    (void)cudaGetLastError();
    *ptr = nullptr;
    return B200_ALLOCATION_FAILED;
  }
  return B200_SUCCESS;
}
int b200_host_free_pinned(void* ptr)
{
  B200_CUDA_TRY(cudaFreeHost(ptr), B200_DEALLOCATION_FAILED);
  return B200_SUCCESS;
}

int b200_field_bytes(int field) { return 4 * field_limbs(field); }

int b200_curve_scalar_field(int curve)
{
  switch (curve) {
  case B200_CURVE_BN254_G1: case B200_CURVE_BN254_G2: return B200_FIELD_BN254_FR;
  case B200_CURVE_BLS12_381_G1: case B200_CURVE_BLS12_381_G2: return B200_FIELD_BLS12_381_FR;
  case B200_CURVE_BLS12_377_G1: case B200_CURVE_BLS12_377_G2: return B200_FIELD_BLS12_377_FR;
  case B200_CURVE_BW6_761_G1: case B200_CURVE_BW6_761_G2: return B200_FIELD_BLS12_377_FQ;
  case B200_CURVE_GRUMPKIN: return B200_FIELD_BN254_FQ;
  default: return -1;
  }
}
static int curve_coord_bytes(int curve)
{
  switch (curve) {
  case B200_CURVE_BN254_G1: case B200_CURVE_GRUMPKIN: return 32;
  case B200_CURVE_BN254_G2: return 64;
  case B200_CURVE_BLS12_381_G1: case B200_CURVE_BLS12_377_G1: return 48;
  case B200_CURVE_BLS12_381_G2: case B200_CURVE_BLS12_377_G2: return 96;
  case B200_CURVE_BW6_761_G1: case B200_CURVE_BW6_761_G2: return 96;
  default: return 0;
  }
}
int b200_curve_affine_bytes(int curve) { return 2 * curve_coord_bytes(curve); }
int b200_curve_projective_bytes(int curve) { return 3 * curve_coord_bytes(curve); }

}
```

### include/icicle_b200.h

```cpp
#ifndef ICICLE_B200_H
#define ICICLE_B200_H

#include <stddef.h>
#include <stdint.h>

#if defined(__GNUC__)
#define B200_API __attribute__((visibility("default")))
#else
#define B200_API
#endif

#ifdef __cplusplus
extern "C" {
#endif

enum {
  B200_SUCCESS = 0,
  B200_INVALID_DEVICE = 1,
  B200_OUT_OF_MEMORY = 2,
  B200_INVALID_POINTER = 3,
  B200_ALLOCATION_FAILED = 4,
  B200_DEALLOCATION_FAILED = 5,
  B200_COPY_FAILED = 6,
  B200_SYNCHRONIZATION_FAILED = 7,
  B200_STREAM_CREATION_FAILED = 8,
  B200_STREAM_DESTRUCTION_FAILED = 9,
  B200_API_NOT_IMPLEMENTED = 10,
  B200_INVALID_ARGUMENT = 11,
  B200_UNKNOWN_ERROR = 14
};

typedef enum {
  B200_FIELD_BN254_FR = 0,
  B200_FIELD_BN254_FQ = 1,
  B200_FIELD_BLS12_381_FR = 2,
  B200_FIELD_BLS12_381_FQ = 3,
  B200_FIELD_BLS12_377_FR = 4,
  B200_FIELD_BLS12_377_FQ = 5,
  B200_FIELD_BW6_761_FQ = 6,
  B200_FIELD_STARK252 = 7,
  B200_FIELD_BABYBEAR = 8,
  B200_FIELD_KOALABEAR = 9,
  B200_FIELD_M31 = 10,
  B200_FIELD_GOLDILOCKS = 11,
  B200_FIELD_BABYBEAR_EXT4 = 12,
  B200_FIELD_KOALABEAR_EXT4 = 13,
  B200_FIELD_COUNT
} b200_field_t;

typedef enum {
  B200_CURVE_BN254_G1 = 0,
  B200_CURVE_BN254_G2 = 1,
  B200_CURVE_BLS12_381_G1 = 2,
  B200_CURVE_BLS12_381_G2 = 3,
  B200_CURVE_BLS12_377_G1 = 4,
  B200_CURVE_BLS12_377_G2 = 5,
  B200_CURVE_BW6_761_G1 = 6,
  B200_CURVE_BW6_761_G2 = 7,
  B200_CURVE_GRUMPKIN = 8,
  B200_CURVE_COUNT
} b200_curve_t;

B200_API int b200_get_device_count(int* count);
B200_API int b200_set_device(int device_id);
B200_API int b200_malloc(void** ptr, size_t bytes);
B200_API int b200_malloc_async(void** ptr, size_t bytes, void* stream);
B200_API int b200_free(void* ptr);
B200_API int b200_free_async(void* ptr, void* stream);
B200_API int b200_get_available_memory(size_t* total, size_t* free_bytes);
B200_API int b200_memset(void* ptr, int value, size_t bytes);
B200_API int b200_memset_async(void* ptr, int value, size_t bytes, void* stream);
B200_API int b200_copy_to_device(void* dst, const void* src, size_t bytes, void* stream, int is_async);
B200_API int b200_copy_to_host(void* dst, const void* src, size_t bytes, void* stream, int is_async);
B200_API int b200_copy_device_to_device(void* dst, const void* src, size_t bytes, void* stream, int is_async);
B200_API int b200_synchronize(void* stream);
B200_API int b200_create_stream(void** stream);
B200_API int b200_destroy_stream(void* stream);
B200_API int b200_host_alloc_pinned(void** ptr, size_t bytes);
B200_API int b200_host_free_pinned(void* ptr);
B200_API int b200_field_bytes(int field);
B200_API int b200_curve_scalar_field(int curve);
B200_API int b200_curve_affine_bytes(int curve);
B200_API int b200_curve_projective_bytes(int curve);

typedef struct {
  void* stream;
  int precompute_factor;
  int c;
  int bitsize;
  int batch_size;
  uint8_t are_points_shared_in_batch;
  uint8_t are_scalars_on_device;
  uint8_t are_scalars_montgomery_form;
  uint8_t are_points_on_device;
  uint8_t are_points_montgomery_form;
  uint8_t are_results_on_device;
  uint8_t is_async;
  uint8_t reserved;
  int ext_large_bucket_factor;
  int ext_nof_chunks;
  int ext_is_big_triangle;
} b200_msm_config;

B200_API void b200_msm_default_config(b200_msm_config* cfg);
B200_API int b200_msm(int curve, const void* scalars, const void* bases, int msm_size, const b200_msm_config* cfg, void* results);
B200_API int b200_msm_precompute_bases(int curve, const void* input_bases, int nof_bases, const b200_msm_config* cfg, void* output_bases);
B200_API int b200_msm_choose_c(int curve, int msm_size, const b200_msm_config* cfg);
B200_API int b200_msm_pair_levels(int curve, int msm_size, const b200_msm_config* cfg);
B200_API int b200_msm_pipeline_schedule(int msm_size, uint32_t* sizes, int max_chunks);

enum { B200_NTT_FORWARD = 0, B200_NTT_INVERSE = 1 };
enum { B200_NN = 0, B200_NR = 1, B200_RN = 2, B200_RR = 3, B200_NM = 4, B200_MN = 5 };
enum { B200_NTT_ALG_AUTO = 0, B200_NTT_ALG_RADIX2 = 1, B200_NTT_ALG_MIXED_RADIX = 2 };

typedef struct {
  void* stream;
  const void* coset_gen;
  int batch_size;
  uint8_t columns_batch;
  uint8_t are_inputs_on_device;
  uint8_t are_outputs_on_device;
  uint8_t is_async;
  int ordering;
  int ext_ntt_algorithm;
  int ext_fast_twiddles;
} b200_ntt_config;

B200_API void b200_ntt_default_config(b200_ntt_config* cfg);
B200_API int b200_ntt_init_domain(int field, const void* primitive_root, void* stream);
B200_API int b200_ntt_release_domain(int field);
B200_API int b200_ntt_get_root_of_unity_from_domain(int field, uint64_t logn, void* rou_out);
B200_API int b200_ntt(int field, const void* input, int size, int dir, const b200_ntt_config* cfg, void* output);
B200_API int b200_ntt_extension(int field, const void* input, int size, int dir, const b200_ntt_config* cfg, void* output);
B200_API int b200_ecntt(int curve, const void* input, int size, int dir, const b200_ntt_config* cfg, void* output);

typedef struct {
  void* stream;
  uint8_t is_a_on_device;
  uint8_t is_b_on_device;
  uint8_t is_result_on_device;
  uint8_t is_async;
  int batch_size;
  uint8_t columns_batch;
  uint8_t reserved[3];
} b200_vec_ops_config;

typedef enum {
  B200_VEC_ADD = 0,
  B200_VEC_SUB = 1,
  B200_VEC_MUL = 2,
  B200_VEC_ACCUMULATE = 3,
  B200_SCALAR_ADD_VEC = 4,
  B200_SCALAR_SUB_VEC = 5,
  B200_SCALAR_MUL_VEC = 6
} b200_vec_op_t;

B200_API void b200_vec_ops_default_config(b200_vec_ops_config* cfg);
B200_API int b200_vec_op(int field, int op, const void* a, const void* b, uint64_t size, const b200_vec_ops_config* cfg, void* out);
B200_API int b200_ext_mixed_mul(int ext_field, const void* a, const void* b, uint64_t size, const b200_vec_ops_config* cfg, void* out);
B200_API int b200_vector_inv(int field, const void* a, uint64_t size, const b200_vec_ops_config* cfg, void* out);
B200_API int b200_vector_div(int field, const void* a, const void* b, uint64_t size, const b200_vec_ops_config* cfg, void* out);
B200_API int b200_vector_sum(int field, const void* a, uint64_t size, const b200_vec_ops_config* cfg, void* out);
B200_API int b200_vector_product(int field, const void* a, uint64_t size, const b200_vec_ops_config* cfg, void* out);
B200_API int b200_highest_non_zero_idx(int field, const void* a, uint64_t size, const b200_vec_ops_config* cfg, int64_t* out_idx);
B200_API int b200_poly_eval(int field, const void* coeffs, uint64_t coeffs_size, const void* domain, uint64_t domain_size,
                            const b200_vec_ops_config* cfg, void* evals);
B200_API int b200_poly_division(int field, const void* numerator, uint64_t numerator_size, const void* denominator, uint64_t denominator_size,
                                const b200_vec_ops_config* cfg, void* q_out, uint64_t q_size, void* r_out, uint64_t r_size);
B200_API int b200_convert_montgomery(int field, const void* in, uint64_t size, int is_into, const b200_vec_ops_config* cfg, void* out);
B200_API int b200_bit_reverse(int field, const void* in, uint64_t size, const b200_vec_ops_config* cfg, void* out);
B200_API int b200_matrix_transpose(int field, const void* in, uint32_t rows, uint32_t cols, const b200_vec_ops_config* cfg, void* out);
B200_API int b200_slice(int field, const void* in, uint64_t offset, uint64_t stride, uint64_t size_in, uint64_t size_out,
               const b200_vec_ops_config* cfg, void* out);
B200_API int b200_affine_convert_montgomery(int curve, const void* in, uint64_t n, int is_into, const b200_vec_ops_config* cfg, void* out);
B200_API int b200_projective_convert_montgomery(int curve, const void* in, uint64_t n, int is_into, const b200_vec_ops_config* cfg, void* out);

B200_API int b200_ec_sum(int curve, const void* points, int n, const b200_vec_ops_config* cfg, void* out);

B200_API int b200_msm_multi_gpu(int curve, const void* scalars, const void* bases, int msm_size, const b200_msm_config* cfg, void* results,
                                int n_devices, const int* device_ids);
B200_API int b200_ntt_multi_gpu(int field, const void* input, int size, int dir, const b200_ntt_config* cfg, void* output,
                                int n_devices, const int* device_ids);
B200_API int b200_ntt_dist_phase1(int field, void* slab, int a_log, int b_log, int n_ranks, int rank, int dir, void* stream);
B200_API int b200_ntt_dist_phase2(int field, const void* received, void* out_slab, int a_log, int b_log, int n_ranks, int rank, int dir, void* stream);
B200_API void b200_shard_range(uint64_t total, int parts, int index, uint64_t* begin, uint64_t* count);

B200_API long long b200_get_launch_count(void);
B200_API void b200_set_profiling(int on);
B200_API int b200_get_last_profile(char* names_out, int names_cap, float* ms_out, int max_stages);

B200_API int b200_set_tuning(const char* name, int value);
B200_API int b200_get_tuning(const char* name);
B200_API int b200_trim_scratch(size_t keep_bytes);

B200_API const char* b200_version(void);

#ifdef __cplusplus
}
#endif
#endif
```

Measured before the change: 345.3 million.

## Add memory-aware MSM window grouping planner to bound accumulation scratch

Result: no change. 345.3 million, median of 6 (+0.0%).

```diff
diff --git a/icicle_b200/api.py b/icicle_b200/api.py
--- a/icicle_b200/api.py
+++ b/icicle_b200/api.py
@@ -236,6 +236,14 @@
     return lib.b200_msm_pair_levels(int(curve), int(msm_size), C.byref(cfg))
 
 
+def msm_plan_groups(curve, msm_size, avail_bytes=None, c=0, config=None):
+    cfg = (config or MSMConfig(c=c))._c()
+    lv, g, peak = C.c_int(0), C.c_int(0), C.c_ulonglong(0)
+    check(lib.b200_msm_plan_groups(int(curve), int(msm_size), C.byref(cfg), -1 if avail_bytes is None else int(avail_bytes),
+                                   C.byref(lv), C.byref(g), C.byref(peak)), "msm_plan_groups")
+    return lv.value, g.value, peak.value
+
+
 def shard_range(total, parts, index):
     b, c = C.c_uint64(0), C.c_uint64(0)
     lib.b200_shard_range(int(total), int(parts), int(index), C.byref(b), C.byref(c))
diff --git a/icicle_b200/capi.py b/icicle_b200/capi.py
--- a/icicle_b200/capi.py
+++ b/icicle_b200/capi.py
@@ -72,6 +72,7 @@
     "b200_ec_sum": (_i, [_i, _vp, _i, C.POINTER(VecOpsConfigC), _vp]),
     "b200_msm_choose_c": (_i, [_i, _i, C.POINTER(MsmConfigC)]),
     "b200_msm_pair_levels": (_i, [_i, _i, C.POINTER(MsmConfigC)]),
+    "b200_msm_plan_groups": (_i, [_i, _i, C.POINTER(MsmConfigC), C.c_longlong, C.POINTER(_i), C.POINTER(_i), C.POINTER(C.c_ulonglong)]),
     "b200_msm_pipeline_schedule": (_i, [_i, C.POINTER(C.c_uint32), _i]),
     "b200_ntt_default_config": (None, [C.POINTER(NttConfigC)]),
     "b200_ntt_init_domain": (_i, [_i, _vp, _vp]),
diff --git a/icicle_b200/csrc/common.cuh b/icicle_b200/csrc/common.cuh
--- a/icicle_b200/csrc/common.cuh
+++ b/icicle_b200/csrc/common.cuh
@@ -26,6 +26,7 @@
 enum Tune : int {
   T_MSM_PAIR_LEVELS = 0, T_MSM_CHUNK_TARGET, T_MSM_NO_WIDE_LOADS, T_MSM_PIPELINE_MIN, T_MSM_PIPELINE_CHUNKS, T_MSM_NO_PIPELINE,
   T_MSM_STAGING_MB, T_MSM_SORT, T_NTT_GEOM, T_NTT31_OFF, T_NTT_COLUMNS_STRIDED, T_NTT_MAXR, T_NTT_TILES, T_NTT_MAXS, T_NTT31_TMA_OFF, T_COPIER_THREADS,
+  T_MSM_GROUPS,
   T_COUNT
 };
 int tune(Tune k);
@@ -120,8 +121,9 @@
 
 struct StageTimer {
   static constexpr int MAX_STAGES = 64;
-  cudaEvent_t ev[MAX_STAGES + 1];
-  const char* names[MAX_STAGES];
+  static constexpr int MAX_MARKS = 512;
+  cudaEvent_t ev[MAX_MARKS + 1];
+  const char* names[MAX_MARKS];
   int n = 0;
   bool on = false;
   cudaStream_t s = nullptr;
diff --git a/icicle_b200/csrc/msm.cu b/icicle_b200/csrc/msm.cu
--- a/icicle_b200/csrc/msm.cu
+++ b/icicle_b200/csrc/msm.cu
@@ -7,6 +7,7 @@
   extern "C" int b200_msm_precompute_entry_##ID(const void*, int, const b200_msm_config*, void*) __attribute__((weak)); \
   extern "C" int b200_msm_plan_c_entry_##ID(int, const b200_msm_config*) __attribute__((weak));                         \
   extern "C" int b200_msm_plan_levels_entry_##ID(int, const b200_msm_config*) __attribute__((weak));                    \
+  extern "C" int b200_msm_plan_groups_entry_##ID(int, const b200_msm_config*, long long, int*, int*, unsigned long long*) __attribute__((weak)); \
   extern "C" int b200_ec_sum_entry_##ID(const void*, int, const b200_vec_ops_config*, void*) __attribute__((weak));       \
   extern "C" int b200_ecntt_entry_##ID(const void*, int, int, const b200_ntt_config*, void*, const uint32_t*, const uint32_t*, int) __attribute__((weak));
 DECL(0) DECL(1) DECL(2) DECL(3) DECL(4) DECL(5) DECL(6) DECL(8)
@@ -109,4 +110,14 @@
 #undef CALL
 }
 
+__attribute__((visibility("default"))) int b200_msm_plan_groups(int curve, int msm_size, const b200_msm_config* cfg, long long avail_bytes,
+                                                                int* levels, int* groups, unsigned long long* peak_bytes)
+{
+  if (!cfg || !levels || !groups || !peak_bytes) return B200_INVALID_POINTER;
+  if (msm_size <= 0) return B200_INVALID_ARGUMENT;
+#define CALL(TU) return b200_msm_plan_groups_entry_##TU(msm_size, cfg, avail_bytes, levels, groups, peak_bytes)
+  ALL_CASES(CALL)
+#undef CALL
 }
+
+}
diff --git a/icicle_b200/csrc/msm_impl.cuh b/icicle_b200/csrc/msm_impl.cuh
--- a/icicle_b200/csrc/msm_impl.cuh
+++ b/icicle_b200/csrc/msm_impl.cuh
@@ -50,9 +50,22 @@
   uint32_t bm_buckets;
 };
 
+struct MsmGroup {
+  uint32_t m0, gm, nwg;
+};
+inline MsmGroup msm_group(const MsmPlan& pl, int g, int groups)
+{
+  MsmGroup gr;
+  gr.m0 = (uint32_t)((uint64_t)g * pl.nbm / groups);
+  gr.gm = (uint32_t)((uint64_t)(g + 1) * pl.nbm / groups) - gr.m0;
+  const uint32_t tail = std::min<uint32_t>(std::max<uint32_t>(pl.nwin % pl.nbm, gr.m0), gr.m0 + gr.gm) - gr.m0;
+  gr.nwg = (uint32_t)(pl.nwin / pl.nbm) * gr.gm + tail;
+  return gr;
+}
+
 template <class S>
 __global__ void __launch_bounds__(256) k_digits(
-  const uint32_t* __restrict__ scalars, uint32_t n, uint32_t batch_local, MsmPlan pl, bool scalars_mont, bool shared_points,
+  const uint32_t* __restrict__ scalars, uint32_t n, uint32_t batch_local, MsmPlan pl, MsmGroup gr, bool scalars_mont, bool shared_points,
   uint32_t* __restrict__ keys, uint32_t* __restrict__ vals, uint32_t sentinel)
 {
   uint64_t g = (uint64_t)blockIdx.x * blockDim.x + threadIdx.x;
@@ -62,7 +75,7 @@
   if (scalars_mont) s = s.from_mont();
   const uint32_t c = pl.c, half = 1u << (c - 1), full = 1u << c;
   uint32_t carry = 0;
-  const uint64_t ent_base = (uint64_t)b * pl.nwin * n;
+  const uint64_t ent_base = (uint64_t)b * gr.nwg * n;
   const uint32_t pt_base = shared_points ? 0u : b * n * pl.pf;
   for (int w = 0; w < pl.nwin; w++) {
     const uint32_t lsb = w * c;
@@ -86,10 +99,11 @@
       neg = 0;
       carry = 0;
     }
-    const uint32_t j = w / pl.nbm, bm = w % pl.nbm;
+    const uint32_t j = w / pl.nbm, lm = w % pl.nbm - gr.m0;
+    if (lm >= gr.gm) continue;
     uint32_t key = sentinel;
-    if (mag) key = (b * pl.nbm + bm) * half + (mag - 1);
-    const uint64_t e = ent_base + (uint64_t)w * n + i;
+    if (mag) key = (b * gr.gm + lm) * half + (mag - 1);
+    const uint64_t e = ent_base + (uint64_t)(j * gr.gm + lm) * n + i;
     keys[e] = key;
     vals[e] = (pt_base + i * pl.pf + j) | (neg ? SIGN_BIT : 0u);
   }
@@ -97,7 +111,7 @@
 
 template <class S>
 __global__ void __launch_bounds__(256) k_digits_rank(
-  const uint32_t* __restrict__ scalars, uint32_t n, uint32_t batch_local, MsmPlan pl, bool scalars_mont, uint32_t* __restrict__ keys,
+  const uint32_t* __restrict__ scalars, uint32_t n, uint32_t batch_local, MsmPlan pl, MsmGroup gr, bool scalars_mont, uint32_t* __restrict__ keys,
   uint32_t* __restrict__ ranks, uint32_t* __restrict__ cnt)
 {
   uint64_t g = (uint64_t)blockIdx.x * blockDim.x + threadIdx.x;
@@ -107,7 +121,7 @@
   if (scalars_mont) s = s.from_mont();
   const uint32_t c = pl.c, half = 1u << (c - 1), full = 1u << c;
   uint32_t carry = 0;
-  const uint64_t ent_base = (uint64_t)b * pl.nwin * n;
+  const uint64_t ent_base = (uint64_t)b * gr.nwg * n;
   for (int w = 0; w < pl.nwin; w++) {
     const uint32_t lsb = w * c;
     uint32_t raw = 0;
@@ -130,13 +144,14 @@
       neg = 0;
       carry = 0;
     }
-    const uint32_t bm = w % pl.nbm;
+    const uint32_t j = w / pl.nbm, lm = w % pl.nbm - gr.m0;
+    if (lm >= gr.gm) continue;
     uint32_t key = SORT_DROPPED, rk = 0;
     if (mag) {
-      key = (b * pl.nbm + bm) * half + (mag - 1);
+      key = (b * gr.gm + lm) * half + (mag - 1);
       rk = atomicAdd(cnt + key, 1u) | neg;
     }
-    const uint64_t e = ent_base + (uint64_t)w * n + i;
+    const uint64_t e = ent_base + (uint64_t)(j * gr.gm + lm) * n + i;
     keys[e] = key;
     ranks[e] = rk;
   }
@@ -453,6 +468,121 @@
   return levels;
 }
 
+inline bool msm_use_cub(uint64_t max_ent) { return tune(T_MSM_SORT) == 1 || (tune(T_MSM_SORT) != 2 && max_ent > (1ull << 25)); }
+
+constexpr uint32_t PAIR_J = 32, INV_G = 64;
+
+struct AccSizes {
+  uint64_t ent;
+  uint64_t nb;
+  int levels;
+  uint64_t cap[10];
+  uint64_t tree_total;
+  uint32_t slice;
+  uint64_t slices;
+  uint64_t bytes;
+};
+
+inline AccSizes acc_sizes(uint64_t ent, uint64_t nb, int levels, bool use_cub, size_t coord_bytes, int sms)
+{
+  AccSizes a;
+  a.ent = ent;
+  a.nb = nb;
+  a.levels = levels;
+  a.cap[0] = ent;
+  for (int l = 0; l < levels; l++) a.cap[l + 1] = a.cap[l] / 2 + nb + 1;
+  const uint64_t tail = a.cap[levels];
+  a.slice = (uint32_t)std::min<uint64_t>(128, std::max<uint64_t>(8, tail / ((uint64_t)sms * 2048)));
+  a.slices = (tail + a.slice - 1) / a.slice;
+  const uint64_t slots = 2 * a.slices, slots2 = 2 * ((slots + 15) / 16) + 2;
+  uint64_t b = 16 * ent;
+  b += ((nb + 1) / SCAN_BLOCK + 1) * 4;
+  b += (slots + slots2) * (8 + 4 * coord_bytes);
+  if (!use_cub) b += 2 * (nb + 1) * 4;
+  a.tree_total = 0;
+  if (levels > 0) {
+    uint64_t cap_max = a.cap[0];
+    for (int l = 1; l < levels; l++) cap_max = std::max(cap_max, a.cap[l]);
+    uint64_t m = (((cap_max + 1) / 2 + (uint64_t)PAIR_J * PAIR_THREADS - 1) / ((uint64_t)PAIR_J * PAIR_THREADS)) * PAIR_THREADS;
+    for (;;) {
+      a.tree_total += m;
+      if (m <= INV_G) break;
+      m = (m + INV_G - 1) / INV_G;
+    }
+    b += 3 * (nb + 1) * 4;
+    for (int l = 1; l <= std::min(levels, 2); l++) b += a.cap[l] * (2 * coord_bytes + 4);
+    b += (a.cap[0] / 2 + 1) * coord_bytes;
+    b += 2 * a.tree_total * coord_bytes;
+  }
+  a.bytes = b;
+  return a;
+}
+
+struct GroupPlan {
+  int chunk;
+  int groups;
+  int levels;
+  AccSizes acc;
+  uint64_t peak;
+};
+
+inline GroupPlan group_plan(uint32_t n, const MsmPlan& pl, int chunk, int groups, int levels, size_t coord_bytes, int sms)
+{
+  GroupPlan p;
+  p.chunk = chunk;
+  p.groups = groups;
+  p.levels = levels;
+  uint32_t nwg = 0, gm = 0;
+  for (int g = 0; g < groups; g++) {
+    const MsmGroup gr = msm_group(pl, g, groups);
+    nwg = std::max(nwg, gr.nwg);
+    gm = std::max(gm, gr.gm);
+  }
+  p.acc = acc_sizes((uint64_t)n * nwg * chunk, ((uint64_t)gm * chunk) << (pl.c - 1), levels,
+                    msm_use_cub((uint64_t)n * pl.nwin * chunk), coord_bytes, sms);
+  p.peak = p.acc.bytes + ((((uint64_t)pl.nbm * chunk) << (pl.c - 1)) * 4 * coord_bytes);
+  return p;
+}
+
+constexpr int MAX_AUTO_GROUPS = 1;
+inline GroupPlan plan_groups(uint32_t n, const MsmPlan& pl, int chunk, size_t coord_bytes, uint64_t avail, int sms)
+{
+  const int levels = choose_pair_levels((uint64_t)n * pl.nwin * chunk, ((uint64_t)pl.nbm * chunk) << (pl.c - 1));
+  if (tune(T_MSM_GROUPS) >= 1) {
+    const int g = std::min(tune(T_MSM_GROUPS), pl.nbm);
+    return group_plan(n, pl, g > 1 ? 1 : chunk, g, levels, coord_bytes, sms);
+  }
+  const uint64_t margin = avail / 16 + (256ull << 20);
+  const uint64_t budget = avail > margin ? avail - margin : 0;
+  if (levels > 0) {
+    GroupPlan p = group_plan(n, pl, chunk, 1, levels, coord_bytes, sms);
+    if (p.peak <= budget) return p;
+    for (int g = (chunk > 1) ? 1 : 2; g <= std::min(pl.nbm, MAX_AUTO_GROUPS); g++) {
+      p = group_plan(n, pl, 1, g, levels, coord_bytes, sms);
+      if (p.peak <= budget) return p;
+    }
+  }
+  return group_plan(n, pl, chunk, 1, 0, coord_bytes, sms);
+}
+
+inline uint64_t msm_avail_bytes()
+{
+  size_t free_b = 0, total_b = 0;
+  if (cudaMemGetInfo(&free_b, &total_b) != cudaSuccess) {
+    (void)cudaGetLastError();
+    return 0;
+  }
+  uint64_t avail = free_b;
+  if (cudaMemPool_t pool = scratch_pool()) {
+    unsigned long long reserved = 0, used = 0;
+    if (cudaMemPoolGetAttribute(pool, cudaMemPoolAttrReservedMemCurrent, &reserved) == cudaSuccess &&
+        cudaMemPoolGetAttribute(pool, cudaMemPoolAttrUsedMemCurrent, &used) == cudaSuccess && reserved > used)
+      avail += reserved - used;
+    (void)cudaGetLastError();
+  }
+  return avail;
+}
+
 enum : int { MSM_ACC = 1, MSM_RED = 2, MSM_ALL = 3 };
 
 template <class C>
@@ -464,17 +594,17 @@
   constexpr int AW = 2 * F::N, XW = 4 * F::N, PW = 3 * F::N;
   int err;
   const uint64_t ent_per_msm = (uint64_t)n * pl.nwin;
-  int chunk = batch_chunk(n, pl, batch, shared, cfg, (size_t)F::BYTES);
   if ((uint64_t)n * pl.pf >= (1ull << 31) || ent_per_msm >= (1ull << 32)) return B200_INVALID_ARGUMENT;
-
-  const uint64_t max_ent = ent_per_msm * chunk;
+  const bool do_acc = (phases & MSM_ACC) != 0, do_red = (phases & MSM_RED) != 0;
+  const int chunk0 = batch_chunk(n, pl, batch, shared, cfg, (size_t)F::BYTES);
+  GroupPlan plan = do_acc ? plan_groups(n, pl, chunk0, (size_t)F::BYTES, msm_avail_bytes(), num_sms())
+                          : group_plan(n, pl, chunk0, 1, 0, (size_t)F::BYTES, num_sms());
+  const int chunk = plan.chunk, groups = plan.groups;
+  AccSizes& az = plan.acc;
+
   const uint64_t max_modules = (uint64_t)pl.nbm * chunk;
   const uint64_t max_buckets = max_modules << (pl.c - 1);
   if (max_buckets >= 0xfffffff0ull) return B200_INVALID_ARGUMENT;
-
-  const uint64_t target_threads = (uint64_t)num_sms() * 2048;
-  uint32_t slice = (uint32_t)std::min<uint64_t>(128, std::max<uint64_t>(8, max_ent / target_threads));
-  const uint64_t max_slices = (max_ent + slice - 1) / slice;
 
   int chunk_target = 16;
   if (tune(T_MSM_CHUNK_TARGET) >= 0) chunk_target = std::max(10, std::min(22, tune(T_MSM_CHUNK_TARGET)));
@@ -483,32 +613,24 @@
   const uint64_t max_chunks = max_buckets >> chunk_log;
 
   if (ext_bkt && (batch != 1 || chunk != 1)) return B200_INVALID_ARGUMENT;
-  const bool do_acc = (phases & MSM_ACC) != 0, do_red = (phases & MSM_RED) != 0;
   Scratch s_k0, s_k1, s_v0, s_v1, s_cub, s_bkt, s_pkey, s_pflag, s_ppt, s_pkey2, s_pflag2, s_ppt2, s_red0, s_red1, s_cnt0, s_off0;
   ScanScratch scan_sc;
   size_t cub_bytes = 0;
-  const bool use_cub = tune(T_MSM_SORT) == 1 || (tune(T_MSM_SORT) != 2 && max_ent > (1ull << 25));
+  const bool use_cub = msm_use_cub(ent_per_msm * chunk);
   if (do_acc) {
-    if ((err = s_k0.alloc(max_ent * 4, s))) return err;
-    if ((err = s_k1.alloc(max_ent * 4, s))) return err;
-    if ((err = s_v0.alloc(max_ent * 4, s))) return err;
-    if ((err = s_v1.alloc(max_ent * 4, s))) return err;
+    if ((err = s_k0.alloc(az.ent * 4, s))) return err;
+    if ((err = s_k1.alloc(az.ent * 4, s))) return err;
+    if ((err = s_v0.alloc(az.ent * 4, s))) return err;
+    if ((err = s_v1.alloc(az.ent * 4, s))) return err;
     if (use_cub) {
       cub::DoubleBuffer<uint32_t> dk(s_k0.as<uint32_t>(), s_k1.as<uint32_t>()), dv(s_v0.as<uint32_t>(), s_v1.as<uint32_t>());
-      cub::DeviceRadixSort::SortPairs(nullptr, cub_bytes, dk, dv, (int64_t)max_ent, 0, 32, s);
+      cub::DeviceRadixSort::SortPairs(nullptr, cub_bytes, dk, dv, (int64_t)az.ent, 0, 32, s);
       if ((err = s_cub.alloc(cub_bytes, s))) return err;
     } else {
-      if ((err = s_cnt0.alloc((size_t)(max_buckets + 1) * 4, s))) return err;
-      if ((err = s_off0.alloc((size_t)(max_buckets + 1) * 4, s))) return err;
-    }
-    if ((err = scan_sc.prepare(max_buckets + 1, s))) return err;
-    if ((err = s_pkey.alloc(max_slices * 2 * 4, s))) return err;
-    if ((err = s_pflag.alloc(max_slices * 2 * 4, s))) return err;
-    if ((err = s_ppt.alloc(max_slices * 2 * XW * 4, s))) return err;
-    const uint64_t max_slots2 = 2 * ((max_slices * 2 + 15) / 16) + 2;
-    if ((err = s_pkey2.alloc(max_slots2 * 4, s))) return err;
-    if ((err = s_pflag2.alloc(max_slots2 * 4, s))) return err;
-    if ((err = s_ppt2.alloc(max_slots2 * XW * 4, s))) return err;
+      if ((err = s_cnt0.alloc((size_t)(az.nb + 1) * 4, s))) return err;
+      if ((err = s_off0.alloc((size_t)(az.nb + 1) * 4, s))) return err;
+    }
+    if ((err = scan_sc.prepare(az.nb + 1, s))) return err;
   }
   if (!ext_bkt && (err = s_bkt.alloc(max_buckets * XW * 4, s))) return err;
   uint32_t* const bkt = ext_bkt ? ext_bkt : s_bkt.as<uint32_t>();
@@ -517,61 +639,54 @@
     if ((err = s_red1.alloc(std::max<uint64_t>(max_chunks / 2 + 1, 1) * XW * 4, s))) return err;
   }
 
-  int levels = do_acc ? choose_pair_levels(max_ent, max_buckets) : 0;
-  constexpr uint32_t PAIR_J = 32, INV_G = 64;
-  const uint32_t nb_max = (uint32_t)max_buckets;
-  uint64_t cap[10];
-  cap[0] = max_ent;
-  for (int l = 0; l < levels; l++) cap[l + 1] = cap[l] / 2 + nb_max + 1;
+  int levels = do_acc ? az.levels : 0;
   Scratch s_off[2], s_cnt, s_lvl[2], s_lkey[2], s_pbuf, s_tree, s_tpre;
-  uint64_t tree_m[8];
-  int tree_levels = 0;
-  uint64_t tree_total = 0;
   if (levels > 0) {
-    uint64_t cap_max = cap[0];
-    for (int l = 1; l < levels; l++) cap_max = std::max(cap_max, cap[l]);
-    uint64_t m = (((cap_max + 1) / 2 + (uint64_t)PAIR_J * PAIR_THREADS - 1) / ((uint64_t)PAIR_J * PAIR_THREADS)) * PAIR_THREADS;
-    for (;;) {
-      tree_m[tree_levels++] = m;
-      tree_total += m;
-      if (m <= INV_G) break;
-      m = (m + INV_G - 1) / INV_G;
-    }
     bool ok = true;
     for (int b = 0; b < 2 && ok; b++) {
-      ok = ok && !s_off[b].alloc(((size_t)nb_max + 1) * 4, s);
+      ok = ok && !s_off[b].alloc(((size_t)az.nb + 1) * 4, s);
       if (b < levels) {
-        ok = ok && !s_lvl[b].alloc((size_t)cap[b + 1] * AW * 4, s);
-        ok = ok && !s_lkey[b].alloc((size_t)cap[b + 1] * 4, s);
+        ok = ok && !s_lvl[b].alloc((size_t)az.cap[b + 1] * AW * 4, s);
+        ok = ok && !s_lkey[b].alloc((size_t)az.cap[b + 1] * 4, s);
       }
     }
-    ok = ok && !s_cnt.alloc(((size_t)nb_max + 1) * 4, s) &&
-         !s_pbuf.alloc(((size_t)cap[0] / 2 + 1) * F::BYTES, s) && !s_tree.alloc((size_t)tree_total * F::BYTES, s) &&
-         !s_tpre.alloc((size_t)tree_total * F::BYTES, s);
+    ok = ok && !s_cnt.alloc(((size_t)az.nb + 1) * 4, s) &&
+         !s_pbuf.alloc(((size_t)az.cap[0] / 2 + 1) * F::BYTES, s) && !s_tree.alloc((size_t)az.tree_total * F::BYTES, s) &&
+         !s_tpre.alloc((size_t)az.tree_total * F::BYTES, s);
     if (!ok) {
       levels = 0;
       for (int b = 0; b < 2; b++) { s_off[b].release(); s_lvl[b].release(); s_lkey[b].release(); }
       s_cnt.release(); s_pbuf.release(); s_tree.release(); s_tpre.release();
-    }
-  }
-  if (levels > 0) {
-    uint32_t sl = (uint32_t)std::min<uint64_t>(128, std::max<uint64_t>(8, cap[levels] / target_threads));
-    while ((cap[levels] + sl - 1) / sl > max_slices) sl++;
-    slice = sl;
+      az = acc_sizes(az.ent, az.nb, 0, use_cub, (size_t)F::BYTES, num_sms());
+    }
+  }
+  const uint32_t slice = az.slice;
+  if (do_acc) {
+    const uint64_t slots = 2 * az.slices, slots2 = 2 * ((slots + 15) / 16) + 2;
+    if ((err = s_pkey.alloc(slots * 4, s))) return err;
+    if ((err = s_pflag.alloc(slots * 4, s))) return err;
+    if ((err = s_ppt.alloc(slots * XW * 4, s))) return err;
+    if ((err = s_pkey2.alloc(slots2 * 4, s))) return err;
+    if ((err = s_pflag2.alloc(slots2 * 4, s))) return err;
+    if ((err = s_ppt2.alloc(slots2 * XW * 4, s))) return err;
   }
 
   for (int b0 = 0; b0 < batch; b0 += chunk) {
     const int bl = std::min(chunk, batch - b0);
-    const uint64_t n_ent = ent_per_msm * bl;
     const uint32_t n_modules = (uint32_t)pl.nbm * bl;
     const uint64_t n_buckets = (uint64_t)n_modules << (pl.c - 1);
-    const uint32_t sentinel = (uint32_t)n_buckets;
     const uint32_t* sc = (const uint32_t*)d_scal + (uint64_t)b0 * n * S::N;
     const uint32_t* pts = pts_m + (shared ? 0 : (uint64_t)b0 * n * pl.pf * AW);
     const bool pts_wide = (((uintptr_t)pts) & 31u) == 0 && (F::BYTES % 32 == 0) && tune(T_MSM_NO_WIDE_LOADS) <= 0;
 
     if (do_acc) {
-    const uint32_t nb = (uint32_t)n_buckets;
+    B200_CUDA_TRY(cudaMemsetAsync(bkt, 0, n_buckets * XW * 4, s), B200_UNKNOWN_ERROR);
+    for (int g = 0; g < groups; g++) {
+    const MsmGroup gr = msm_group(pl, g, groups);
+    const uint64_t n_ent = (uint64_t)n * gr.nwg * bl;
+    const uint32_t nb = (uint32_t)(((uint64_t)gr.gm * bl) << (pl.c - 1));
+    const uint32_t sentinel = nb;
+    uint32_t* const gbkt = bkt + ((uint64_t)gr.m0 << (pl.c - 1)) * XW;
     const uint32_t* sorted_k;
     const uint32_t* sorted_v;
     const uint32_t* n_live = nullptr;
@@ -580,7 +695,7 @@
     if (use_cub) {
       uint64_t th = (uint64_t)n * bl;
       k_digits<S><<<(unsigned)((th + 255) / 256), 256, 0, s>>>(
-        sc, n, (uint32_t)bl, pl, cfg->are_scalars_montgomery_form, shared, s_k0.as<uint32_t>(), s_v0.as<uint32_t>(), sentinel); B200_LAUNCHED(1);
+        sc, n, (uint32_t)bl, pl, gr, cfg->are_scalars_montgomery_form, shared, s_k0.as<uint32_t>(), s_v0.as<uint32_t>(), sentinel); B200_LAUNCHED(1);
       B200_CUDA_TRY(cudaGetLastError(), B200_UNKNOWN_ERROR);
       prof.mark("digits");
       cub::DoubleBuffer<uint32_t> dk(s_k0.as<uint32_t>(), s_k1.as<uint32_t>()), dv(s_v0.as<uint32_t>(), s_v1.as<uint32_t>());
@@ -596,11 +711,11 @@
       B200_CUDA_TRY(cudaMemsetAsync(s_cnt0.p, 0, ((size_t)nb + 1) * 4, s), B200_UNKNOWN_ERROR);
       uint64_t th = (uint64_t)n * bl;
       k_digits_rank<S><<<(unsigned)((th + 255) / 256), 256, 0, s>>>(
-        sc, n, (uint32_t)bl, pl, cfg->are_scalars_montgomery_form, s_k0.as<uint32_t>(), s_v0.as<uint32_t>(), s_cnt0.as<uint32_t>()); B200_LAUNCHED(1);
+        sc, n, (uint32_t)bl, pl, gr, cfg->are_scalars_montgomery_form, s_k0.as<uint32_t>(), s_v0.as<uint32_t>(), s_cnt0.as<uint32_t>()); B200_LAUNCHED(1);
       B200_CUDA_TRY(cudaGetLastError(), B200_UNKNOWN_ERROR);
       prof.mark("digits");
       if ((err = exclusive_scan_u32(s_cnt0.as<uint32_t>(), off_first, (uint64_t)nb + 1, scan_sc, s))) return err;
-      k_scatter<<<(unsigned)((n_ent + 255) / 256), 256, 0, s>>>(s_k0.as<uint32_t>(), s_v0.as<uint32_t>(), n_ent, n, (uint32_t)pl.nwin, (uint32_t)pl.nbm,
+      k_scatter<<<(unsigned)((n_ent + 255) / 256), 256, 0, s>>>(s_k0.as<uint32_t>(), s_v0.as<uint32_t>(), n_ent, n, gr.nwg, gr.gm,
                                                                (uint32_t)pl.pf, shared, off_first, s_k1.as<uint32_t>(), s_v1.as<uint32_t>()); B200_LAUNCHED(1);
       B200_CUDA_TRY(cudaGetLastError(), B200_UNKNOWN_ERROR);
       sorted_k = s_k1.as<uint32_t>();
@@ -609,12 +724,11 @@
       acc_sentinel = 0xffffffffu;
       prof.mark("sort");
     }
-    B200_CUDA_TRY(cudaMemsetAsync(bkt, 0, n_buckets * XW * 4, s), B200_UNKNOWN_ERROR);
     uint64_t n_slices;
     if (levels == 0) {
       n_slices = (n_ent + slice - 1) / slice;
       k_accumulate<F, false><<<(unsigned)((n_slices + MSM_THREADS - 1) / MSM_THREADS), MSM_THREADS, 0, s>>>(
-        sorted_k, sorted_v, n_ent, n_live, slice, acc_sentinel, pts, bkt, s_pkey.as<uint32_t>(),
+        sorted_k, sorted_v, n_ent, n_live, slice, acc_sentinel, pts, gbkt, s_pkey.as<uint32_t>(),
         s_pflag.as<uint32_t>(), s_ppt.as<uint32_t>(), n_slices, pts_wide); B200_LAUNCHED(1);
       B200_CUDA_TRY(cudaGetLastError(), B200_UNKNOWN_ERROR);
     } else {
@@ -623,7 +737,7 @@
       const uint32_t *lk = sorted_k, *lp = pts;
       uint64_t lcap = 0;
       uint4* pbuf = s_pbuf.as<uint4>();
-      const uint64_t pcap = cap[0] / 2 + 1;
+      const uint64_t pcap = az.cap[0] / 2 + 1;
       for (int l = 0; l < levels; l++) {
         uint32_t* off_c = s_off[l & 1].as<uint32_t>();
         uint32_t* off_n = s_off[(l + 1) & 1].as<uint32_t>();
@@ -636,7 +750,7 @@
         uint32_t* tpre = s_tpre.as<uint32_t>();
         uint32_t* out_p = s_lvl[l & 1].as<uint32_t>();
         uint32_t* out_k = s_lkey[l & 1].as<uint32_t>();
-        const uint64_t ocap = cap[(l & 1) + 1];
+        const uint64_t ocap = az.cap[(l & 1) + 1];
         const bool last = (l + 1 == levels);
         if (l == 0) {
           PairSrc<F, true> src = {lk, sorted_v, lp, 0, pts_wide};
@@ -683,7 +797,7 @@
       prof.mark("pair_levels");
       n_slices = (capl + slice - 1) / slice;
       k_accumulate<F, true><<<(unsigned)((n_slices + MSM_THREADS - 1) / MSM_THREADS), MSM_THREADS, 0, s>>>(
-        lk, nullptr, 0, s_off[levels & 1].as<uint32_t>() + nb, slice, 0xffffffffu, lp, bkt, s_pkey.as<uint32_t>(),
+        lk, nullptr, 0, s_off[levels & 1].as<uint32_t>() + nb, slice, 0xffffffffu, lp, gbkt, s_pkey.as<uint32_t>(),
         s_pflag.as<uint32_t>(), s_ppt.as<uint32_t>(), n_slices, true); B200_LAUNCHED(1);
       B200_CUDA_TRY(cudaGetLastError(), B200_UNKNOWN_ERROR);
     }
@@ -696,17 +810,18 @@
       while (n_slots > 512) {
         const uint64_t nt = (n_slots + seg - 1) / seg;
         k_reduce_partials<F><<<(unsigned)((nt + MSM_THREADS - 1) / MSM_THREADS), MSM_THREADS, 0, s>>>(
-          ik, ifl, ipt, n_slots, seg, ok, ofl, opt, nt, bkt); B200_LAUNCHED(1);
+          ik, ifl, ipt, n_slots, seg, ok, ofl, opt, nt, gbkt); B200_LAUNCHED(1);
         B200_CUDA_TRY(cudaGetLastError(), B200_UNKNOWN_ERROR);
         std::swap(ik, ok);
         std::swap(ifl, ofl);
         std::swap(ipt, opt);
         n_slots = 2 * nt;
       }
-      k_resolve<F><<<(unsigned)((n_slots + MSM_THREADS - 1) / MSM_THREADS), MSM_THREADS, 0, s>>>(ik, ifl, ipt, n_slots, bkt); B200_LAUNCHED(1);
+      k_resolve<F><<<(unsigned)((n_slots + MSM_THREADS - 1) / MSM_THREADS), MSM_THREADS, 0, s>>>(ik, ifl, ipt, n_slots, gbkt); B200_LAUNCHED(1);
       B200_CUDA_TRY(cudaGetLastError(), B200_UNKNOWN_ERROR);
     }
     prof.mark("resolve");
+    }
     }
     if (!do_red) continue;
     const uint64_t n_chunks = n_buckets >> chunk_log;
diff --git a/icicle_b200/csrc/msm_inst.cu b/icicle_b200/csrc/msm_inst.cu
--- a/icicle_b200/csrc/msm_inst.cu
+++ b/icicle_b200/csrc/msm_inst.cu
@@ -65,14 +65,27 @@
 {
   return make_plan<ThisCurve>(msm_size, cfg).c;
 }
-__attribute__((visibility("hidden"))) int B200_CAT(b200_msm_plan_levels_entry_, B200_MSM_CURVE)(int msm_size, const b200_msm_config* cfg)
+static GroupPlan plan_of(int msm_size, const b200_msm_config* cfg, long long avail_bytes)
 {
   const MsmPlan pl = make_plan<ThisCurve>(msm_size, cfg);
   const int batch = cfg->batch_size > 0 ? cfg->batch_size : 1;
   const bool shared = cfg->are_points_shared_in_batch || batch == 1;
   const int chunk = batch_chunk((uint32_t)msm_size, pl, batch, shared, cfg, (size_t)ThisCurve::Base::BYTES);
-  const uint64_t max_ent = (uint64_t)msm_size * pl.nwin * chunk;
-  const uint64_t max_buckets = ((uint64_t)pl.nbm * chunk) << (pl.c - 1);
-  return choose_pair_levels(max_ent, max_buckets);
+  const bool on_device = avail_bytes < 0;
+  return plan_groups((uint32_t)msm_size, pl, chunk, (size_t)ThisCurve::Base::BYTES, on_device ? msm_avail_bytes() : (uint64_t)avail_bytes,
+                     on_device ? num_sms() : 132 );
+}
+__attribute__((visibility("hidden"))) int B200_CAT(b200_msm_plan_levels_entry_, B200_MSM_CURVE)(int msm_size, const b200_msm_config* cfg)
+{
+  return plan_of(msm_size, cfg, -1).levels;
+}
+__attribute__((visibility("hidden"))) int B200_CAT(b200_msm_plan_groups_entry_, B200_MSM_CURVE)(
+  int msm_size, const b200_msm_config* cfg, long long avail_bytes, int* levels, int* groups, unsigned long long* peak_bytes)
+{
+  const GroupPlan p = plan_of(msm_size, cfg, avail_bytes);
+  *levels = p.levels;
+  *groups = p.groups;
+  *peak_bytes = p.peak;
+  return B200_SUCCESS;
 }
 }
diff --git a/icicle_b200/csrc/msm_sort.cuh b/icicle_b200/csrc/msm_sort.cuh
--- a/icicle_b200/csrc/msm_sort.cuh
+++ b/icicle_b200/csrc/msm_sort.cuh
@@ -109,7 +109,7 @@
 }
 
 static __global__ void __launch_bounds__(256) k_scatter(const uint32_t* __restrict__ keys0, const uint32_t* __restrict__ rank0, uint64_t n_ent,
-                                                        uint32_t n, uint32_t nwin, uint32_t nbm, uint32_t pf, bool shared_points,
+                                                        uint32_t n, uint32_t nwg, uint32_t gm, uint32_t pf, bool shared_points,
                                                         const uint32_t* __restrict__ off, uint32_t* __restrict__ keys1, uint32_t* __restrict__ vals1)
 {
   const uint64_t e = (uint64_t)blockIdx.x * blockDim.x + threadIdx.x;
@@ -119,8 +119,8 @@
   const uint32_t r = rank0[e];
   const uint32_t i = (uint32_t)(e % n);
   const uint32_t bw = (uint32_t)(e / n);
-  const uint32_t b = bw / nwin, w = bw % nwin;
-  const uint32_t val = ((shared_points ? 0u : b * n * pf) + i * pf + w / nbm) | (r & SORT_SIGN_BIT);
+  const uint32_t b = bw / nwg, wr = bw % nwg;
+  const uint32_t val = ((shared_points ? 0u : b * n * pf) + i * pf + wr / gm) | (r & SORT_SIGN_BIT);
   const uint32_t pos = off[key] + (r & ~SORT_SIGN_BIT);
   keys1[pos] = key;
   vals1[pos] = val;
diff --git a/icicle_b200/csrc/runtime.cu b/icicle_b200/csrc/runtime.cu
--- a/icicle_b200/csrc/runtime.cu
+++ b/icicle_b200/csrc/runtime.cu
@@ -21,7 +21,8 @@
 namespace {
   const char* const kTuneNames[b200::T_COUNT] = {
     "msm_pair_levels", "msm_chunk_target", "msm_no_wide_loads", "msm_pipeline_min", "msm_pipeline_chunks", "msm_no_pipeline",
-    "msm_staging_mb", "msm_sort", "ntt_geom", "ntt31_off", "ntt_columns_strided", "ntt_maxr", "ntt_tiles", "ntt_maxs", "ntt31_tma_off", "copier_threads"};
+    "msm_staging_mb", "msm_sort", "ntt_geom", "ntt31_off", "ntt_columns_strided", "ntt_maxr", "ntt_tiles", "ntt_maxs", "ntt31_tma_off", "copier_threads",
+    "msm_groups"};
   std::atomic<int> g_tune[b200::T_COUNT];
   struct TuneInit {
     TuneInit()
@@ -87,7 +88,7 @@
   }
   void StageTimer::mark(const char* name)
   {
-    if (!on || n >= MAX_STAGES) return;
+    if (!on || n >= MAX_MARKS) return;
     names[n] = name;
     cudaEventCreate(&ev[n + 1]);
     cudaEventRecord(ev[n + 1], s);
@@ -99,11 +100,20 @@
     cudaEventSynchronize(ev[n]);
     std::lock_guard<std::mutex> lk(g_prof_mu);
     g_prof_what = what;
-    g_prof_n = n;
+    g_prof_n = 0;
     for (int i = 0; i < n; i++) {
-      cudaEventElapsedTime(&g_prof_ms[i], ev[i], ev[i + 1]);
-      strncpy(g_prof_names[i], names[i], 31);
-      g_prof_names[i][31] = 0;
+      float ms = 0.f;
+      cudaEventElapsedTime(&ms, ev[i], ev[i + 1]);
+      int k = 0;
+      while (k < g_prof_n && strncmp(g_prof_names[k], names[i], 31)) k++;
+      if (k == g_prof_n) {
+        if (k == MAX_STAGES) continue;
+        strncpy(g_prof_names[k], names[i], 31);
+        g_prof_names[k][31] = 0;
+        g_prof_ms[k] = 0.f;
+        g_prof_n++;
+      }
+      g_prof_ms[k] += ms;
     }
     for (int i = 0; i <= n; i++) cudaEventDestroy(ev[i]);
     on = false;
diff --git a/include/icicle_b200.h b/include/icicle_b200.h
--- a/include/icicle_b200.h
+++ b/include/icicle_b200.h
@@ -107,6 +107,8 @@
 B200_API int b200_msm_precompute_bases(int curve, const void* input_bases, int nof_bases, const b200_msm_config* cfg, void* output_bases);
 B200_API int b200_msm_choose_c(int curve, int msm_size, const b200_msm_config* cfg);
 B200_API int b200_msm_pair_levels(int curve, int msm_size, const b200_msm_config* cfg);
+B200_API int b200_msm_plan_groups(int curve, int msm_size, const b200_msm_config* cfg, long long avail_bytes, int* levels, int* groups,
+                                  unsigned long long* peak_bytes);
 B200_API int b200_msm_pipeline_schedule(int msm_size, uint32_t* sizes, int max_chunks);
 
 enum { B200_NTT_FORWARD = 0, B200_NTT_INVERSE = 1 };
```
